# Tung-I/Dual-awareness-Attention-for-Few-shot-Object-Detection

Measured on AMD Instinct MI355X. Metric: query-images/sec (res50, way=2, shot=3, bs=4 per GPU, train-mode forward), higher is better.
Workload: dtype f32 (operands, accumulation, results; multiplies as an exact bf16x3 split, six bf16 MFMA products each)

## Files before the change

dual-awareness-attention-for-few-shot-object-detection_amd/csrc/igemm.hip:

```cpp
#include "common.h"
#include "../../include/dana_hip_debug.h"
#include <stdlib.h>
#include <atomic>

namespace {

typedef float f32x16 __attribute__((ext_vector_type(16)));
typedef unsigned int u32x4 __attribute__((ext_vector_type(4)));

struct IgemmParams {
  const float* A;
  const float* Bw;
  float* C;
  const float* scale;
  const float* shift;
  const float* residual;
  const float* mask;
  long ldm;
  int M, N, K;
  int IH, IW, OH, OW, Cin, KH, KW, stride, pad;
  int M0, IH1, IW1, OH1, OW1, pix1;
  float* C1;
  const float* residual1;
  long ldc1, ldr1;
  int lda, ldb;
  long ldc, ldr;
  long batch_a, batch_b, batch_c;
  unsigned a_bytes, b_bytes;
  float alpha;
  int relu;
  int vec_io;
  int vec_ss;
  int tiles_m, tiles_n;
  const float* A2;
  int lda2, IH2, IW2, stride2, K1;
  int IH21, IW21, pix21;
  int bpre;
  const void* Bw2;
  const float* scale2;
  const float* shift2;
  int N2, relu2;
  unsigned a2_bytes;
  int apre, a_rows;
  int res_sample, res_h, res_w, res_oh, res_ow;
  unsigned res_bytes;
  unsigned long long* trace;
};

constexpr int BK = 32;
constexpr int LDS_LD = 36;
constexpr unsigned OOB = 0x80000000u;

__device__ __forceinline__ int xcd_remap(int bid, int nwg) {
  const int q = nwg / 8, r = nwg % 8;
  const int xcd = bid % 8, local = bid / 8;
  return (xcd < r ? xcd * (q + 1) : r * (q + 1) + (xcd - r) * q) + local;
}

__device__ __forceinline__ float4 ldg_b128(__amdgpu_buffer_rsrc_t r, unsigned off) {
  u32x4 v = __builtin_amdgcn_raw_buffer_load_b128(r, (int)off, 0, 0);
  return *(float4*)&v;
}

template <int BM, int BN, int STEM>
__global__ void __launch_bounds__(256, 2) igemm_f32_kernel(IgemmParams p) {
  constexpr int TM = BM / 64, TN = BN / 64;
  constexpr int RA = BM / 32, RB = BN / 32;
  constexpr int CLD = BN + 4;
  extern __shared__ __attribute__((aligned(16))) float smem[];
  float* As = smem;
  float* Bs = smem + 2 * BM * LDS_LD;

  const int tid = threadIdx.x;
  const int lane = tid & 63, wave = tid >> 6;
  const int wm = wave >> 1, wn = wave & 1;
  const int li = lane & 31, lh = lane >> 5;

  const int vid = xcd_remap((int)(blockIdx.z * gridDim.x + blockIdx.x), (int)(gridDim.x * gridDim.z));
  const int zb = vid / (int)gridDim.x;
  const int tile = vid - zb * (int)gridDim.x;
  const int tm_idx = tile / p.tiles_n, tn_idx = tile % p.tiles_n;
  const int m0 = tm_idx * BM, n0 = tn_idx * BN;
  const float* Ab = p.A + (long)zb * p.batch_a;
  const float* Bb = p.Bw + (long)zb * p.batch_b;
  float* Cb = p.C + (long)zb * p.batch_c;
  const __amdgpu_buffer_rsrc_t ra_src = __builtin_amdgcn_make_buffer_rsrc((void*)Ab, 0, (int)p.a_bytes, 0x00020000);
  const __amdgpu_buffer_rsrc_t rb_src = __builtin_amdgcn_make_buffer_rsrc((void*)Bb, 0, (int)p.b_bytes, 0x00020000);

  const int c4 = tid & 7;
  const int r0 = tid >> 3;
  unsigned a_off[RA];
  unsigned long long a_mask[RA];
  bool a_seg1[RA];
#pragma unroll
  for (int j = 0; j < RA; ++j) {
    const int m = m0 + r0 + 32 * j;
    const bool ok = m < p.M;
    const bool s1 = ok && m >= p.M0;
    a_seg1[j] = s1;
    const int mm = ok ? (s1 ? m - p.M0 : m) : 0;
    const int IH = s1 ? p.IH1 : p.IH, IW = s1 ? p.IW1 : p.IW, OW = s1 ? p.OW1 : p.OW;
    const int ohw = (s1 ? p.OH1 : p.OH) * OW;
    const int img = mm / ohw, rem = mm - img * ohw;
    const int oh = rem / OW, ow = rem - oh * OW;
    const int ih0 = oh * p.stride - p.pad, iw0 = ow * p.stride - p.pad;
    const int pix = (s1 ? p.pix1 : 0) + (img * IH + ih0) * IW;
    unsigned long long mask = 0;
    if (STEM) {
      const int iw = iw0 + c4;
      if (ok && c4 < 7 && iw >= 0 && iw < IW)
        for (int kh = 0; kh < 7; ++kh)
          if (ih0 + kh >= 0 && ih0 + kh < IH) mask |= 1ull << kh;
      a_off[j] = (unsigned)((pix + iw) * 16);
    } else {
      if (ok)
        for (int kh = 0; kh < p.KH; ++kh)
          for (int kw = 0; kw < p.KW; ++kw)
            if (ih0 + kh >= 0 && ih0 + kh < IH && iw0 + kw >= 0 && iw0 + kw < IW)
              mask |= 1ull << (kh * p.KW + kw);
      a_off[j] = (unsigned)(((pix + iw0) * p.lda + c4 * 4) * 4);
    }
    a_mask[j] = mask;
  }
  unsigned b_off[RB];
#pragma unroll
  for (int j = 0; j < RB; ++j) {
    const int n = n0 + r0 + 32 * j;
    b_off[j] = n < p.N ? (unsigned)((n * p.ldb + c4 * 4) * 4) : OOB;
  }

  float4 ra0[RA], rb0[RB], ra1[RA], rb1[RB];
  auto load_tile = [&](int kt, float4(&ra)[RA], float4(&rb)[RB]) {
    const int k0 = kt * BK;
    const bool kok = (k0 + c4 * 4) < p.K;
    int tap;
    unsigned delta, delta1;
    if (STEM) {
      tap = kt;
      delta = (unsigned)(kt * p.IW * 16);
      delta1 = (unsigned)(kt * p.IW1 * 16);
    } else {
      tap = k0 / p.Cin;
      const int cin0 = k0 - tap * p.Cin;
      const int kh = tap / p.KW, kw = tap - kh * p.KW;
      delta = (unsigned)(((kh * p.IW + kw) * p.lda + cin0) * 4);
      delta1 = (unsigned)(((kh * p.IW1 + kw) * p.lda + cin0) * 4);
    }
#pragma unroll
    for (int j = 0; j < RA; ++j) {
      const bool ok = kok && ((a_mask[j] >> tap) & 1ull);
      ra[j] = ldg_b128(ra_src, ok ? a_off[j] + (a_seg1[j] ? delta1 : delta) : OOB);
    }
#pragma unroll
    for (int j = 0; j < RB; ++j) rb[j] = ldg_b128(rb_src, (kok && b_off[j] != OOB) ? b_off[j] + k0 * 4 : OOB);
  };
  auto store_tile = [&](int buf, const float4(&ra)[RA], const float4(&rb)[RB]) {
    float* as = As + buf * BM * LDS_LD;
    float* bs = Bs + buf * BN * LDS_LD;
#pragma unroll
    for (int j = 0; j < RA; ++j) *(float4*)(as + (r0 + 32 * j) * LDS_LD + c4 * 4) = ra[j];
#pragma unroll
    for (int j = 0; j < RB; ++j) *(float4*)(bs + (r0 + 32 * j) * LDS_LD + c4 * 4) = rb[j];
  };

  f32x16 acc[TM][TN];
#pragma unroll
  for (int i = 0; i < TM; ++i)
#pragma unroll
// ... 215 lines not shown
             : __builtin_amdgcn_make_buffer_rsrc((void*)(p.residual ? (seg1 ? p.residual1 : p.residual) + mrel * ld_r : p.A), 0,
                                                 p.residual ? rows_valid * ldr4 : 0, 0x00020000);
    const __amdgpu_buffer_rsrc_t rc_msk = __builtin_amdgcn_make_buffer_rsrc(
        (void*)(p.mask ? p.mask + (long)m0 * p.ldm : p.A), 0, p.mask ? rows_valid * ldm4 : 0, 0x00020000);
    const int lrow = wm * (BM / 2) + 4 * lh;
    unsigned vo_c[TN], vo_r[TN], vo_m[TN];
#pragma unroll
    for (int j = 0; j < TN; ++j) {
      const bool nok = ncol[j] < p.N;
      vo_c[j] = nok ? (unsigned)(lrow * ldc4 + ncol[j] * 4) : OOB;
      vo_r[j] = nok ? (unsigned)((RSMP ? 0 : lrow * ldr4) + ncol[j] * 4) : OOB;
      vo_m[j] = nok ? (unsigned)(lrow * ldm4 + ncol[j] * 4) : OOB;
    }
    auto run = [&](auto res_c, auto relu_c, auto mask_c) {
      constexpr bool RES = decltype(res_c)::value != 0, RELU = decltype(relu_c)::value != 0, MASK = decltype(mask_c)::value != 0;
      constexpr int HI = (MASK || HALVES) ? 1 : TM;
#pragma unroll
      for (int i0 = 0; i0 < TM; i0 += HI) {
        float res[RES ? HI : 1][TN][16], msk[MASK ? HI : 1][TN][16];
#pragma unroll
        for (int ii = 0; ii < HI; ++ii)
#pragma unroll
          for (int j = 0; j < TN; ++j)
#pragma unroll
            for (int r = 0; r < 16; ++r) {
              const int rt = (i0 + ii) * 32 + (r & 3) + 8 * (r >> 2);
              if constexpr (RES && RSMP)
                res[ii][j][r] = __builtin_bit_cast(float, __builtin_amdgcn_raw_buffer_load_b32(rc_res, (int)(vo_r[j] + rtab[lrow + rt]), 0, 0));
              else if constexpr (RES)
                res[ii][j][r] = __builtin_bit_cast(float, __builtin_amdgcn_raw_buffer_load_b32(rc_res, (int)(vo_r[j] + (unsigned)(rt * ldr4)), 0, 0));
              if constexpr (MASK)
                msk[ii][j][r] = __builtin_bit_cast(float, __builtin_amdgcn_raw_buffer_load_b32(rc_msk, (int)(vo_m[j] + (unsigned)(rt * ldm4)), 0, 0));
            }
#pragma unroll
        for (int ii = 0; ii < HI; ++ii)
#pragma unroll
          for (int j = 0; j < TN; ++j)
#pragma unroll
            for (int r = 0; r < 16; ++r) {
              const int rt = (i0 + ii) * 32 + (r & 3) + 8 * (r >> 2);
              float v = acc[i0 + ii][j][r] * scv[j] + shv[j];
              if constexpr (RES) v += res[ii][j][r];
              if constexpr (RELU) v = fmaxf(v, 0.f);
              if constexpr (MASK) v = msk[ii][j][r] > 0.f ? v : 0.f;
              __builtin_amdgcn_raw_buffer_store_b32(__builtin_bit_cast(unsigned, v), rc_dst, (int)(vo_c[j] + (unsigned)(rt * ldc4)), 0, 0);
            }
      }
    };
    if (WITH_MASK && p.mask) {
      if (p.residual) {
        if (p.relu) run(IC<1>{}, IC<1>{}, IC<1>{});
        else run(IC<1>{}, IC<0>{}, IC<1>{});
      } else {
        if (p.relu) run(IC<0>{}, IC<1>{}, IC<1>{});
        else run(IC<0>{}, IC<0>{}, IC<1>{});
      }
    } else if (p.residual) {
      if (p.relu) run(IC<1>{}, IC<1>{}, IC<0>{});
      else run(IC<1>{}, IC<0>{}, IC<0>{});
    } else {
      if (p.relu) run(IC<0>{}, IC<1>{}, IC<0>{});
      else run(IC<0>{}, IC<0>{}, IC<0>{});
    }
  } else {
#pragma unroll
    for (int i = 0; i < TM; ++i)
#pragma unroll
      for (int j = 0; j < TN; ++j)
#pragma unroll
        for (int r = 0; r < 16; ++r) {
          const int m = m0 + wm * (BM / 2) + i * 32 + (r & 3) + 8 * (r >> 2) + 4 * lh;
          if (m < p.M && ncol[j] < p.N) {
            const bool s1 = m >= p.M0;
            float v = acc[i][j][r] * scv[j] + shv[j];
            if (p.residual) v += s1 ? p.residual1[(long)(m - p.M0) * p.ldr1 + ncol[j]] : p.residual[(long)m * p.ldr + ncol[j]];
            if (p.relu) v = fmaxf(v, 0.f);
            if (p.mask && !(p.mask[(long)m * p.ldm + ncol[j]] > 0.f)) v = 0.f;
            (s1 ? p.C1 + (long)(m - p.M0) * p.ldc1 : Cb + (long)m * p.ldc)[ncol[j]] = v;
          }
        }
  }
}

template <int BM, int BN, int STEM, int BPRE = 0, int FUSE = 0, int ELDS = 0, int RSMP = 0>
__device__ __forceinline__ void igemm_split_body(const IgemmParams& p) {
  static_assert(!RSMP || (!STEM && !FUSE && !ELDS), "sampled residual: register epilogue of the plain conv / GEMM forms");
  constexpr int TM = BM / 64, TN = BN / 64;
  constexpr int RA = BM / 64;
  constexpr int RB = BPRE ? (3 * BN * 2 + 255) / 256 : BN / 64;
  constexpr int CLD = BN + 4;
  extern __shared__ __attribute__((aligned(16))) float smem[];
  unsigned* As = (unsigned*)smem;
  unsigned* Bs = As + 2 * 3 * BM * SLD;

  const int tid = threadIdx.x;
  const int lane = tid & 63, wave = tid >> 6;
  const int wm = wave >> 1, wn = wave & 1;
  const int li = lane & 31, lh = lane >> 5;

  const unsigned long long t_start = p.trace ? __builtin_readcyclecounter() : 0ull;
  const unsigned long long w_start = p.trace ? wall_clock64() : 0ull;
  const int vid = xcd_remap((int)(blockIdx.z * gridDim.x + blockIdx.x), (int)(gridDim.x * gridDim.z));
  const int zb = vid / (int)gridDim.x;
  const int tile = vid - zb * (int)gridDim.x;
  const int tm_idx = tile / p.tiles_n, tn_idx = tile % p.tiles_n;
  const int m0 = tm_idx * BM, n0 = tn_idx * BN;
  const float* Ab = p.A + (long)zb * p.batch_a;
  const float* Bb = p.Bw + (long)zb * p.batch_b;
  float* Cb = p.C + (long)zb * p.batch_c;
  __amdgpu_buffer_rsrc_t ra_src = __builtin_amdgcn_make_buffer_rsrc((void*)Ab, 0, (int)p.a_bytes, 0x00020000);
  const __amdgpu_buffer_rsrc_t rb_src = __builtin_amdgcn_make_buffer_rsrc((void*)Bb, 0, (int)p.b_bytes, 0x00020000);

  int cin_t = STEM ? SBK : p.Cin;
  const int kw_t = STEM ? 2 : p.KW;
  const int kh_t = STEM ? 7 : p.KH;
  const int lda4 = (STEM ? 4 : p.lda) * 4;
  const int kwstep = STEM ? 4 * lda4 : lda4;
  const int c4 = tid & 3;
  const int r0 = tid >> 2;
  const int wcol = ((c4 >> 1) ^ swz(r0)) * 4 + (c4 & 1) * 2;
  const int rcol = (lh ^ swz(li)) * 4;
  const int klim = p.K - c4 * 4;
  constexpr int DEAD = (int)0x80000000;
  unsigned a_off[RA];
  unsigned a_mask[RA];
  int a_dseg[RA];
  unsigned a_off2[RA];
  const bool lin = !STEM && p.KH * p.KW == 1 && p.stride == 1 && p.pad == 0;
#pragma unroll
  for (int j = 0; j < RA; ++j) {
    const int m = m0 + r0 + 64 * j;
    const bool ok = m < p.M;
    const bool s1 = ok && m >= p.M0;
    const int mm = ok ? (s1 ? m - p.M0 : m) : 0;
    if (lin && !p.A2) {
      a_off[j] = (unsigned)(((s1 ? p.pix1 : 0) + mm) * lda4 + c4 * 16);
      a_mask[j] = ok ? 1u : 0u;
      a_dseg[j] = 0;
      a_off2[j] = OOB;
      continue;
    }
    const int IH = s1 ? p.IH1 : p.IH, IW = s1 ? p.IW1 : p.IW, OW = s1 ? p.OW1 : p.OW;
    const int ohw = (s1 ? p.OH1 : p.OH) * OW;
    const int img = mm / ohw, rem = mm - img * ohw;
    const int oh = rem / OW, ow = rem - oh * OW;
    const int ih0 = oh * p.stride - p.pad, iw0 = ow * p.stride - p.pad;
    const int pix = (s1 ? p.pix1 : 0) + (img * IH + ih0) * IW;
    unsigned mask = 0;
    if (STEM) {
      const int lo = ih0 < 0 ? -ih0 : 0, hi = IH - ih0 < 7 ? IH - ih0 : 7;
      const int iwa = iw0 + c4, iwb = iw0 + 4 + c4;
      const unsigned cv = ((iwa >= 0 && iwa < IW) ? 0x1555u : 0u) | ((iwb >= 0 && iwb < IW && c4 < 3) ? 0x2aaau : 0u);
      if (ok && hi > lo) mask = ((1u << (2 * hi)) - (1u << (2 * lo))) & cv;
    } else if (ok) {
      unsigned colbits = 0;
      for (int kw = 0; kw < kw_t; ++kw)
        if (iw0 + kw >= 0 && iw0 + kw < IW) colbits |= 1u << kw;
      for (int kh = 0; kh < kh_t; ++kh)
        if (ih0 + kh >= 0 && ih0 + kh < IH) mask |= colbits << (kh * kw_t);
    }
    a_off[j] = STEM ? (unsigned)((pix + iw0 + c4) * lda4) : (unsigned)((pix + iw0) * lda4 + c4 * 16);
    a_mask[j] = mask;
    a_dseg[j] = s1 ? (p.IW1 - p.IW) * lda4 : 0;
    a_off2[j] = (!STEM && p.A2 && ok)
                    ? (unsigned)(((s1 ? p.pix21 : 0) + ((long)img * (s1 ? p.IH21 : p.IH2) + oh * p.stride2) * (s1 ? p.IW21 : p.IW2) +
                                  ow * p.stride2) * p.lda2 * 4 + c4 * 16)
                    : OOB;
  }
  unsigned b_cur[RB];
  int b_lim[RB];
  int b_lds[RB];
#pragma unroll
  for (int j = 0; j < RB; ++j) {
    if constexpr (BPRE) {
      const int q = (tid + 256 * j < 6 * BN) ? tid + 256 * j : tid;
      const int pl = q / (2 * BN), rem = q - pl * (2 * BN);
      const int row = rem >> 1, half = rem & 1;
      const int n = n0 + row;
      b_cur[j] = (unsigned)((((long)pl * p.N + n) * SBK + half * 8) * 2);
      b_lim[j] = n < p.N ? (p.K + SBK - 1) / SBK * SBK : DEAD;
      b_lds[j] = (pl * BN + row) * SLD + (half ^ swz(row)) * 4;
    } else {
      const int n = n0 + r0 + 64 * j;
      b_cur[j] = (unsigned)((n * p.ldb + c4 * 4) * 4);
      b_lim[j] = n < p.N ? klim : DEAD;
      b_lds[j] = 0;
    }
  }
  const unsigned B_STEP = BPRE ? (unsigned)p.N * 3u * SBK * 2u : SBK * 4;

  float4 ra0[RA], rb0[RB], ra1[RA], rb1[RB];
  int lt_k0 = 0, lt_cin = 0, lt_kh = 0, lt_kw = 0;
// ... 481 lines not shown
          *(float4*)(c_base + (long)(qq * RPP) * ld_c) = make_float4(v[0], v[1], v[2], v[3]);
        }
      }
    };
    if (p.mask) {
      if (p.residual) {
        if (p.relu) emit(IC<1>{}, IC<1>{}, IC<1>{});
        else emit(IC<1>{}, IC<0>{}, IC<1>{});
      } else {
        if (p.relu) emit(IC<0>{}, IC<1>{}, IC<1>{});
        else emit(IC<0>{}, IC<0>{}, IC<1>{});
      }
    } else if (p.residual) {
      if (p.relu) emit(IC<1>{}, IC<1>{}, IC<0>{});
      else emit(IC<1>{}, IC<0>{}, IC<0>{});
    } else {
      if (p.relu) emit(IC<0>{}, IC<1>{}, IC<0>{});
      else emit(IC<0>{}, IC<0>{}, IC<0>{});
    }
  } else if (full4) {
#pragma unroll
    for (int q = 0; q < NP; ++q) {
      const int rr = er + q * RPP;
      const int m = m0 + rr;
      if (m < p.M) {
        const float4 a4 = *(const float4*)(Cs + rr * CLD + ec);
        float v[4] = {a4.x * sc[0] + sh[0], a4.y * sc[1] + sh[1], a4.z * sc[2] + sh[2], a4.w * sc[3] + sh[3]};
        float* cp = c_base + (long)(q * RPP) * ld_c;
        if (!one_seg) {
          const bool s1 = m >= p.M0;
          cp = s1 ? p.C1 + (long)(m - p.M0) * p.ldc1 + n : Cb + (long)m * p.ldc + n;
        }
        if (p.residual) {
          v[0] += rres[q].x;
          v[1] += rres[q].y;
          v[2] += rres[q].z;
          v[3] += rres[q].w;
        }
        if (p.relu) {
#pragma unroll
          for (int t = 0; t < 4; ++t) v[t] = fmaxf(v[t], 0.f);
        }
        if (p.mask) {
          const float4 k4 = *(const float4*)(p.mask + (long)m * p.ldm + n);
          v[0] = k4.x > 0.f ? v[0] : 0.f;
          v[1] = k4.y > 0.f ? v[1] : 0.f;
          v[2] = k4.z > 0.f ? v[2] : 0.f;
          v[3] = k4.w > 0.f ? v[3] : 0.f;
        }
        *(float4*)cp = make_float4(v[0], v[1], v[2], v[3]);
      }
    }
  } else {
    for (int q = 0; q < NP; ++q) {
      const int rr = er + q * RPP;
      const int m = m0 + rr;
      if (m >= p.M) break;
      const bool s1 = m >= p.M0;
      float* cp = s1 ? p.C1 + (long)(m - p.M0) * p.ldc1 + n : Cb + (long)m * p.ldc + n;
      const float* rp = s1 ? p.residual1 + (long)(m - p.M0) * p.ldr1 + n : p.residual + (long)m * p.ldr + n;
      for (int t = 0; t < 4; ++t)
        if ((n + t) < p.N) {
          float x = Cs[rr * CLD + ec + t] * sc[t] + sh[t];
          if (p.residual) x += rp[t];
          if (p.relu) x = fmaxf(x, 0.f);
          if (p.mask && !(p.mask[(long)m * p.ldm + n + t] > 0.f)) x = 0.f;
          cp[t] = x;
        }
    }
  }
  if (p.trace && tid == 0) {
    unsigned long long* tr = p.trace + ((long)blockIdx.z * gridDim.x + blockIdx.x) * 8;
    tr[0] = t_start;
    tr[1] = t_loop;
    tr[2] = t_loop_end;
    tr[3] = __builtin_readcyclecounter();
    tr[4] = (unsigned long long)__builtin_amdgcn_s_getreg((31 << 11) | 4) | ((unsigned long long)__builtin_amdgcn_s_getreg((31 << 11) | 20) << 32);
    tr[5] = wall_clock64();
    tr[6] = w_start;
    tr[7] = 0;
  }
}

template <int BM, int BN, int STEM, int BPRE = 0, int FUSE = 0, int ELDS = 0, int RSMP = 0>
__global__ void __launch_bounds__(256, 2) igemm_split_kernel(IgemmParams p) {
  igemm_split_body<BM, BN, STEM, BPRE, FUSE, ELDS, RSMP>(p);
}
template <int STEM, int BPRE, int ELDS, int RSMP = 0>
__global__ void __launch_bounds__(256, 1) __attribute__((amdgpu_num_vgpr(192))) igemm_split_kernel_128(IgemmParams p) {
  igemm_split_body<128, 128, STEM, BPRE, 0, ELDS, RSMP>(p);
}

template <int BN, int NST, int APRE, int DF = 0>
__global__ void __launch_bounds__(256, NST == 2 ? 3 : (NST == 3 ? 2 : 1)) igemm_dma_kernel(IgemmParams p) {
  static_assert(APRE || NST == 2, "fp32 activation rows: two stages");
  static_assert(!DF || (APRE && NST >= 3), "two fragment sets: planes x planes, three or more stages");
  constexpr int BM = 128, TM = 2, TN = BN / 64;
  constexpr int STAGE_B = 3 * (BM + BN) * 32;
  constexpr int NPB = 3 * BN / 32, PB = (NPB + 3) / 4;
  constexpr int NDMA = (APRE ? 3 : 0) + PB;
  constexpr int AHEAD = NST == 2 ? 2 : NST - 1;
  constexpr int RA = BM / 64;
  extern __shared__ __attribute__((aligned(16))) float smem[];
  const int tid = threadIdx.x;
  const int lane = tid & 63, wave = __builtin_amdgcn_readfirstlane(tid >> 6);
  const int wm = wave >> 1, wn = wave & 1;
  const int li = lane & 31, lh = lane >> 5;
  const unsigned long long t_start = p.trace ? __builtin_readcyclecounter() : 0ull;
  const unsigned long long w_start = p.trace ? wall_clock64() : 0ull;
  const int vid = xcd_remap((int)(blockIdx.z * gridDim.x + blockIdx.x), (int)(gridDim.x * gridDim.z));
  const int zb = vid / (int)gridDim.x;
  const int tile = vid - zb * (int)gridDim.x;
  const int tm_idx = tile / p.tiles_n, tn_idx = tile % p.tiles_n;
  const int m0 = tm_idx * BM, n0 = tn_idx * BN;
  float* Cb = p.C + (long)zb * p.batch_c;
  __amdgpu_buffer_rsrc_t ra_src =
      __builtin_amdgcn_make_buffer_rsrc((void*)(p.A + (long)zb * p.batch_a), 0, (int)p.a_bytes, 0x00020000);
  const __amdgpu_buffer_rsrc_t rb_src =
      __builtin_amdgcn_make_buffer_rsrc((void*)(p.Bw + (long)zb * p.batch_b), 0, (int)p.b_bytes, 0x00020000);
  const int nk = (p.K + SBK - 1) / SBK;

  const int prow = lane >> 1, phalf = (lane & 1) ^ ((lane >> 4) & 1);
  const int arow = m0 + 32 * wave + prow;
  const unsigned a_vo = arow < p.M ? (unsigned)(arow * 32 + phalf * 16) : OOB;
  const unsigned a_pstride = (unsigned)p.a_rows * 32u, b_pstride = (unsigned)p.N * 32u;
  unsigned b_vo[PB];
  int b_pl[PB], b_lds[PB];
#pragma unroll
  for (int j = 0; j < PB; ++j) {
    int q = wave + 4 * j;
    if (q >= NPB) q -= 4;
    const int pl = q / (BN / 32), rg = q % (BN / 32);
    const int n = n0 + 32 * rg + prow;
    b_vo[j] = n < p.N ? (unsigned)(n * 32 + phalf * 16) : OOB;
    b_pl[j] = pl;
    b_lds[j] = 3 * BM * 32 + (pl * BN + 32 * rg) * 32;
  }
  typedef __attribute__((address_space(3))) void lds_void;
  typedef __attribute__((address_space(3))) char lds_char;
  lds_char* const lds0 = (lds_char*)(lds_void*)smem;
  auto issue = [&](int t, int stage) {
    const bool live = t < nk;
    lds_char* base = lds0 + stage * STAGE_B;
    if constexpr (APRE) {
      const unsigned av = live ? a_vo : OOB;
      const unsigned sa = (unsigned)t * 3u * a_pstride;
#pragma unroll
      for (int pl = 0; pl < 3; ++pl)
        __builtin_amdgcn_raw_ptr_buffer_load_lds(ra_src, (lds_void*)(base + (pl * BM + 32 * wave) * 32), 16, (int)av,
                                                 (int)(sa + pl * a_pstride), 0, 0);
    }
    const unsigned sb = (unsigned)t * 3u * b_pstride;
#pragma unroll
    for (int j = 0; j < PB; ++j)
      __builtin_amdgcn_raw_ptr_buffer_load_lds(rb_src, (lds_void*)(base + b_lds[j]), 16, (int)(live ? b_vo[j] : OOB),
                                               (int)(sb + b_pl[j] * b_pstride), 0, 0);
  };

  int cin_t = p.Cin;
  const int kw_t = p.KW, kh_t = p.KH;
  const int lda4 = p.lda * 4;
  const int c4 = tid & 3, r0 = tid >> 2;
  const int wcol = ((c4 >> 1) ^ swz(r0)) * 4 + (c4 & 1) * 2;
  const int klim = p.K - c4 * 4;
  constexpr int DEAD = (int)0x80000000;
  unsigned a_off[RA], a_mask[RA], a_off2[RA];
  int a_dseg[RA];
  int lt_k0 = 0, lt_cin = 0, lt_kh = 0, lt_kw = 0;
  unsigned lt_bit = 1u;
  unsigned a_cur[RA];
  int a_lim[RA];
  if constexpr (!APRE) {
    const bool lin = p.KH * p.KW == 1 && p.stride == 1 && p.pad == 0;
#pragma unroll
    for (int j = 0; j < RA; ++j) {
      const int m = m0 + r0 + 64 * j;
      const bool ok = m < p.M;
      const bool s1 = ok && m >= p.M0;
      const int mm = ok ? (s1 ? m - p.M0 : m) : 0;
      if (lin && !p.A2) {
        a_off[j] = (unsigned)(((s1 ? p.pix1 : 0) + mm) * lda4 + c4 * 16);
        a_mask[j] = ok ? 1u : 0u;
        a_dseg[j] = 0;
        a_off2[j] = OOB;
      } else {
        const int IH = s1 ? p.IH1 : p.IH, IW = s1 ? p.IW1 : p.IW, OW = s1 ? p.OW1 : p.OW;
        const int ohw = (s1 ? p.OH1 : p.OH) * OW;
        const int img = mm / ohw, rem = mm - img * ohw;
        const int oh = rem / OW, ow = rem - oh * OW;
        const int ih0 = oh * p.stride - p.pad, iw0 = ow * p.stride - p.pad;
        const int pix = (s1 ? p.pix1 : 0) + (img * IH + ih0) * IW;
        unsigned mask = 0;
        if (ok) {
          unsigned colbits = 0;
          for (int kw = 0; kw < kw_t; ++kw)
            if (iw0 + kw >= 0 && iw0 + kw < IW) colbits |= 1u << kw;
          for (int kh = 0; kh < kh_t; ++kh)
            if (ih0 + kh >= 0 && ih0 + kh < IH) mask |= colbits << (kh * kw_t);
        }
        a_off[j] = (unsigned)((pix + iw0) * lda4 + c4 * 16);
        a_mask[j] = mask;
        a_dseg[j] = s1 ? (p.IW1 - p.IW) * lda4 : 0;
// ... 180 lines not shown
  const unsigned long long t_loop_end = p.trace ? __builtin_readcyclecounter() : 0ull;
  epilogue_regs<BM, BN, (NST == 2 && BN == 128) ? 1 : 0, 0>(p, acc, m0, n0, Cb, wm, wn, li, lh);
  if (p.trace && tid == 0) {
    unsigned long long* tr = p.trace + ((long)blockIdx.z * gridDim.x + blockIdx.x) * 8;
    tr[0] = t_start;
    tr[1] = t_loop;
    tr[2] = t_loop_end;
    tr[3] = __builtin_readcyclecounter();
    tr[4] = (unsigned long long)__builtin_amdgcn_s_getreg((31 << 11) | 4) | ((unsigned long long)__builtin_amdgcn_s_getreg((31 << 11) | 20) << 32);
    tr[5] = wall_clock64();
    tr[6] = w_start;
    tr[7] = 0;
  }
}

template <int NMAX>
__global__ void __launch_bounds__(256)
gemm_skinny_kernel(const float* __restrict__ a, const float* __restrict__ b, float* __restrict__ c,
                   const float* __restrict__ scale, const float* __restrict__ shift, int M, int N, int K, long lda,
                   long ldb, long ldc, float alpha, int relu) {
  const int lane = threadIdx.x & 63;
  const long m = (long)blockIdx.x * 4 + (threadIdx.x >> 6);
  if (m >= M) return;
  float acc[NMAX];
#pragma unroll
  for (int n = 0; n < NMAX; ++n) acc[n] = 0.f;
  const float4* ar = (const float4*)(a + m * lda);
  for (int k4 = lane; k4 < K / 4; k4 += 64) {
    const float4 x = ar[k4];
#pragma unroll
    for (int n = 0; n < NMAX; ++n)
      if (n < N) {
        const float4 w = ((const float4*)(b + n * ldb))[k4];
        acc[n] += x.x * w.x + x.y * w.y + x.z * w.z + x.w * w.w;
      }
  }
#pragma unroll
  for (int n = 0; n < NMAX; ++n) {
#pragma unroll
    for (int o = 32; o > 0; o >>= 1) acc[n] += __shfl_xor(acc[n], o);
  }
  if (lane == 0)
    for (int n = 0; n < N; ++n) {
      float v = acc[n] * alpha * (scale ? scale[n] : 1.f) + (shift ? shift[n] : 0.f);
      if (relu) v = fmaxf(v, 0.f);
      c[m * ldc + n] = v;
    }
}

__global__ void __launch_bounds__(256)
split_weight_kernel(const float* __restrict__ w, long ldw, long batch_w, int n, int k, int kp,
                    unsigned short* __restrict__ out) {
  const int kq = kp / 4;
  const long idx = (long)blockIdx.x * blockDim.x + threadIdx.x;
  if (idx >= (long)n * kq) return;
  const int row = (int)(idx / kq), k4 = (int)(idx - (long)row * kq) * 4;
  const float* src = w + blockIdx.y * batch_w + (long)row * ldw + k4;
  float4 v = make_float4(0.f, 0.f, 0.f, 0.f);
  if (k4 + 3 < k) v = *(const float4*)src;
  else {
    if (k4 < k) v.x = src[0];
    if (k4 + 1 < k) v.y = src[1];
    if (k4 + 2 < k) v.z = src[2];
  }
  uint2 h, m, l;
  split3(v, h, m, l);
  const int ks = k4 / SBK, kk = k4 - ks * SBK;
  unsigned short* o = out + blockIdx.y * 3 * (long)n * kp + (((long)ks * 3) * n + row) * SBK + kk;
  *(uint2*)o = h;
  *(uint2*)(o + (long)n * SBK) = m;
  *(uint2*)(o + 2 * (long)n * SBK) = l;
}

std::atomic<int>& epilogue_mode_cell() {
  static std::atomic<int> cell(0);
  return cell;
}

std::atomic<int> g_last_form(0);
constexpr int form_code(int family, int bm, int bn, int stem, int bpre, int fuse, int elds, int nst, int apre, int df) {
  return family | (bm / 64) << 4 | (bn / 64) << 6 | stem << 8 | bpre << 9 | fuse << 10 | elds << 11 | nst << 12 | apre << 16 | df << 17;
}

template <int BM, int BN, int STEM>
int launch(const IgemmParams& p0, int batch, hipStream_t s) {
  g_last_form.store(form_code(DANA_IGEMM_FAMILY_F32, BM, BN, STEM, 0, 0, 0, 0, 0, 0), std::memory_order_relaxed);
  IgemmParams p = p0;
  p.tiles_m = (p.M + BM - 1) / BM;
  p.tiles_n = (p.N + BN - 1) / BN;
  size_t lds = (size_t)2 * (BM + BN) * LDS_LD * sizeof(float);
  const size_t lds_c = (size_t)BM * (BN + 4) * sizeof(float);
  if (lds_c > lds) lds = lds_c;
  static DeviceOnce attr;
  attr.once([&] { return hipFuncSetAttribute((const void*)igemm_f32_kernel<BM, BN, STEM>, hipFuncAttributeMaxDynamicSharedMemorySize, (int)lds); });
  dim3 grid(p.tiles_m * p.tiles_n, 1, batch);
  igemm_f32_kernel<BM, BN, STEM><<<grid, 256, lds, s>>>(p);
  return 0;
}

template <int BM, int BN, int STEM = 0, int BPRE = 0, int FUSE = 0, int ELDS = 0, int RSMP = 0>
int launch_split(const IgemmParams& p0, int batch, hipStream_t s) {
  if constexpr (BPRE == 0 && FUSE == 0) {
    if (p0.bpre) return launch_split<BM, BN, STEM, 1, 0, ELDS, RSMP>(p0, batch, s);
  }
  if constexpr (ELDS == 0 && FUSE == 0 && RSMP == 0) {
    if (epilogue_mode_cell().load(std::memory_order_relaxed)) return launch_split<BM, BN, STEM, BPRE, 0, 1>(p0, batch, s);
  }
  g_last_form.store(form_code(BM * BN >= 128 * 128 ? DANA_IGEMM_FAMILY_SPLIT_128 : DANA_IGEMM_FAMILY_SPLIT, BM, BN, STEM, BPRE, FUSE ? 1 : 0,
                              ELDS, 0, 0, 0), std::memory_order_relaxed);
  IgemmParams p = p0;
  p.tiles_m = (p.M + BM - 1) / BM;
  p.tiles_n = (p.N + BN - 1) / BN;
  size_t lds = (size_t)2 * 3 * (BM + BN) * SLD * sizeof(unsigned);
  const size_t lds_c = (size_t)BM * (BN + 4) * sizeof(float);
  if (lds_c > lds && ELDS) lds = lds_c;
  if (FUSE && lds < (size_t)4 * 3 * BM * 16 * 2) lds = (size_t)4 * 3 * BM * 16 * 2;
  if (FUSE == 2 || RSMP) lds += (size_t)BM * 4;
  dim3 grid(p.tiles_m * p.tiles_n, 1, batch);
  static DeviceOnce attr;
  if constexpr (BM * BN >= 128 * 128) {
    attr.once([&] { return hipFuncSetAttribute((const void*)igemm_split_kernel_128<STEM, BPRE, ELDS, RSMP>, hipFuncAttributeMaxDynamicSharedMemorySize,
                                (int)lds); });
    igemm_split_kernel_128<STEM, BPRE, ELDS, RSMP><<<grid, 256, lds, s>>>(p);
  } else {
    attr.once([&] { return hipFuncSetAttribute((const void*)igemm_split_kernel<BM, BN, STEM, BPRE, FUSE, ELDS, RSMP>,
                                hipFuncAttributeMaxDynamicSharedMemorySize, (int)lds); });
    igemm_split_kernel<BM, BN, STEM, BPRE, FUSE, ELDS, RSMP><<<grid, 256, lds, s>>>(p);
  }
  return 0;
}

template <int BN, int NST, int APRE, int DF = 0>
int launch_dma(const IgemmParams& p0, int batch, hipStream_t s) {
  g_last_form.store(form_code(DANA_IGEMM_FAMILY_DMA, 128, BN, 0, 1, 0, 0, NST, APRE, DF), std::memory_order_relaxed);
  IgemmParams p = p0;
  p.tiles_m = (p.M + 127) / 128;
  p.tiles_n = (p.N + BN - 1) / BN;
  const size_t lds = (size_t)NST * 3 * (128 + BN) * 32;
  static DeviceOnce attr;
  attr.once([&] { return hipFuncSetAttribute((const void*)igemm_dma_kernel<BN, NST, APRE, DF>, hipFuncAttributeMaxDynamicSharedMemorySize, (int)lds); });
  dim3 grid(p.tiles_m * p.tiles_n, 1, batch);
  igemm_dma_kernel<BN, NST, APRE, DF><<<grid, 256, lds, s>>>(p);
  return 0;
}

std::atomic<int>& mfma_mode_cell() {
  static std::atomic<int> cell(getenv("DANA_MFMA_SPLIT") ? atoi(getenv("DANA_MFMA_SPLIT")) : 1);
  return cell;
}
int env_choice(const char* name, std::initializer_list<int> allowed) {
  const char* e = getenv(name);
  if (!e || !*e) return -1;
  const int v = atoi(e);
  for (int a : allowed)
    if (a == v) return v;
  fprintf(stderr, "libdana_hip: %s=%s is not one of the accepted values; ignored\n", name, e);
  return -1;
}
int dma_kernel_env() {
  static const int v = env_choice("DANA_DMA_KERNEL", {0, 1, 2});
  return v;
}
std::atomic<int>& dma_kernel_cell() {
  static std::atomic<int> cell(dma_kernel_env());
  return cell;
}
int pp_stages_env() {
  static const int v = env_choice("DANA_PP_STAGES", {2, 3, 4, 6, 13, 14});
  return v;
}
std::atomic<int>& pp_stages_cell() {
  static std::atomic<int> cell(pp_stages_env());
  return cell;
}
unsigned long long* g_trace = nullptr;

int dispatch_sampled(const IgemmParams& p, int batch, hipStream_t s) {
  const int mode = mfma_mode_cell().load(std::memory_order_relaxed);
  if (!mode || p.apre || p.mask || p.KH * p.KW > 32 || p.M0 != p.M || epilogue_mode_cell().load(std::memory_order_relaxed)) return -1;
  if (p.N <= 64) return -1;
  if (mode == 3) return launch_split<64, 64, 0, 0, 0, 0, 1>(p, batch, s);
  if (mode == 4) return launch_split<128, 128, 0, 0, 0, 0, 1>(p, batch, s);
  if (p.N <= 256 && p.N % 128 != 0 && p.N % 128 <= 32) return launch_split<64, 64, 0, 0, 0, 0, 1>(p, batch, s);
  const long t128 = (long)((p.M + 127) / 128) * ((p.N + 127) / 128) * batch;
  if (t128 < 100) return launch_split<64, 64, 0, 0, 0, 0, 1>(p, batch, s);
  return launch_split<128, 128, 0, 0, 0, 0, 1>(p, batch, s);
}

int dispatch(const IgemmParams& p, int batch, int stem, hipStream_t s) {
  if (p.res_sample) return stem ? -1 : dispatch_sampled(p, batch, s);
  if (stem) {
    const int smode = mfma_mode_cell().load(std::memory_order_relaxed);
    return smode ? launch_split<128, 64, 1>(p, batch, s) : launch<128, 64, 1>(p, batch, s);
  }
  const int mode = mfma_mode_cell().load(std::memory_order_relaxed);
  if (p.apre) {
    const int pp_env = pp_stages_cell().load(std::memory_order_relaxed);
    const long t128 = (long)((p.M + 127) / 128) * ((p.N + 127) / 128) * batch;
    const int stages = pp_env >= 0 ? pp_env : ((t128 < 400 || p.K >= 1024) ? 13 : 2);
    if (p.N <= 64) return stages == 2 ? launch_dma<64, 2, 1>(p, batch, s) : launch_dma<64, 3, 1>(p, batch, s);
    if (stages == 2) return launch_dma<128, 2, 1>(p, batch, s);
    if (stages == 4) return launch_dma<128, 4, 1>(p, batch, s);
    if (stages == 6) return launch_dma<128, 6, 1>(p, batch, s);
    if (stages == 13) return launch_dma<128, 3, 1, 1>(p, batch, s);
    if (stages == 14) return launch_dma<128, 4, 1, 1>(p, batch, s);
    return launch_dma<128, 3, 1>(p, batch, s);
  }
  if (mode == 1 && p.bpre && !p.mask && p.KH * p.KW <= 32) {
    const int dm_env = dma_kernel_cell().load(std::memory_order_relaxed);
    const int dm = dm_env >= 0 ? dm_env : 1;
    if (dm == 2) return p.N <= 64 ? launch_dma<64, 2, 0>(p, batch, s) : launch_dma<128, 2, 0>(p, batch, s);
    if (dm == 1 && p.N > 64) {
      const long t128 = (long)((p.M + 127) / 128) * ((p.N + 127) / 128) * batch;
      if (t128 >= 600 && p.K <= 192) return launch_dma<128, 2, 0>(p, batch, s);
    }
  }
  if (mode && p.KH * p.KW <= 32) {
    if (mode == 2) return launch_split<128, 64>(p, batch, s);
    if (mode == 3) return launch_split<64, 64>(p, batch, s);
    if (mode == 4) return launch_split<128, 128>(p, batch, s);
    if (mode == 5) return launch_split<64, 128>(p, batch, s);
    if (p.N <= 64) return launch_split<128, 64>(p, batch, s);
    if (mode == 1 && p.N <= 256 && p.N % 128 != 0 && p.N % 128 <= 32) return launch_split<64, 64>(p, batch, s);
    const long t128 = (long)((p.M + 127) / 128) * ((p.N + 127) / 128) * batch;
    if (mode == 1 && t128 < 100) return launch_split<64, 64>(p, batch, s);
    return launch_split<128, 128>(p, batch, s);
  }
  return launch<64, 64, 0>(p, batch, s);
}

int run(IgemmParams& p, int batch, int stem, hipStream_t s) {
  if (p.M0 <= 0 || p.M0 > p.M) p.M0 = p.M;
  if (p.M0 == p.M) {
    p.IH1 = p.IH; p.IW1 = p.IW; p.OH1 = p.OH; p.OW1 = p.OW; p.pix1 = 0;
    p.C1 = p.C; p.ldc1 = p.ldc; p.residual1 = p.residual; p.ldr1 = p.ldr;
  }
  p.trace = g_trace;
  p.vec_io = (p.ldc % 4 == 0) && (((uintptr_t)p.C & 15) == 0) && (p.batch_c % 4 == 0) &&
             (!p.residual || ((p.ldr % 4 == 0) && (((uintptr_t)p.residual & 15) == 0))) &&
             (p.ldc1 % 4 == 0) && (((uintptr_t)p.C1 & 15) == 0) &&
             (!p.residual1 || ((p.ldr1 % 4 == 0) && (((uintptr_t)p.residual1 & 15) == 0)));
  p.vec_ss = (((uintptr_t)p.scale | (uintptr_t)p.shift) & 15) == 0;
  return dispatch(p, batch, stem, s);
}

}

extern "C" {

int dana_set_epilogue_mode(int mode) {
  DANA_CHECK_ARG(mode == 0 || mode == 1, "dana_set_epilogue_mode: 0 (accumulator registers) or 1 (LDS C tile)");
  epilogue_mode_cell().store(mode, std::memory_order_relaxed);
  return DANA_OK;
}
int dana_get_epilogue_mode(void) { return epilogue_mode_cell().load(std::memory_order_relaxed); }

int dana_set_mfma_mode(int mode) {
  DANA_CHECK_ARG(mode == 0 || mode == 1, "dana_set_mfma_mode: mode must be 0 (f32 MFMA) or 1 (bf16x6 split)");
  mfma_mode_cell().store(mode, std::memory_order_relaxed);
  return DANA_OK;
}

int dana_debug_force_tile(int tile) {
  DANA_CHECK_ARG(tile == 0 || (tile >= 2 && tile <= 5), "dana_debug_force_tile: 0 (dispatcher), 2 = 128x64, 3 = 64x64, 4 = 128x128, 5 = 64x128");
  DANA_CHECK_ARG(mfma_mode_cell().load(std::memory_order_relaxed) != 0, "dana_debug_force_tile: split kernel only");
  mfma_mode_cell().store(tile ? tile : 1, std::memory_order_relaxed);
  return DANA_OK;
}

int dana_debug_set_dma_kernel(int v) {
  DANA_CHECK_ARG(v >= -1 && v <= 2, "dana_debug_set_dma_kernel: -1 (environment / default), 0 (split kernel), 1 (measured rule) or 2 (wherever it runs)");
  dma_kernel_cell().store(v < 0 ? dma_kernel_env() : v, std::memory_order_relaxed);
// ... 277 lines not shown
  IgemmParams p;
  memset(&p, 0, sizeof(p));
  p.A = a0;
  p.Bw = weight;
  p.C = out0;
  p.scale = scale;
  p.shift = shift;
  p.residual = residual;
  p.IH = p.OH = oh0;
  p.IW = p.OW = ow0;
  p.M0 = (int)m0;
  p.M = (int)(m0 + m1);
  if (n1) {
    p.IH1 = p.OH1 = oh1;
    p.IW1 = p.OW1 = ow1;
    p.pix1 = (int)m0;
    p.C1 = out1;
    p.IH21 = h1;
    p.IW21 = w1;
    p.pix21 = n0 * h0 * w0;
  }
  p.N = cout;
  p.KH = p.KW = 1;
  p.stride = 1;
  p.pad = 0;
  p.Cin = k0;
  p.K = k0 + k1;
  p.lda = (int)lda0;
  p.ldb = p.K;
  p.a_bytes = (unsigned)a0_bytes;
  p.b_bytes = (unsigned)b_bytes;
  p.bpre = bpre;
  p.A2 = a1;
  p.lda2 = (int)lda1;
  p.IH2 = h0;
  p.IW2 = w0;
  p.stride2 = stride1;
  p.K1 = k1;
  p.a2_bytes = (unsigned)a1_bytes;
  p.ldc = out0_pix_stride > 0 ? out0_pix_stride : cout;
  p.ldr = res_pix_stride > 0 ? res_pix_stride : cout;
  p.ldc1 = n1 ? (out1_pix_stride > 0 ? out1_pix_stride : cout) : p.ldc;
  p.ldr1 = p.ldr;
  p.alpha = 1.f;
  p.relu = (flags & DANA_EPI_RELU) ? 1 : 0;
  p.ldm = cout;
  run(p, 1, 0, (hipStream_t)stream);
  DANA_CHECK_LAUNCH(who);
  return DANA_OK;
}

int dana_conv1x1_cat2_nhwc(const float* a0, long a0_pix_stride, int k0, const float* a1, long a1_pix_stride, int k1,
                           int batch, int h1, int w1, int stride1, const float* weight, float* output,
                           const float* scale, const float* shift, const float* residual, long out_pix_stride,
                           long res_pix_stride, int cout, int flags, dana_stream_t stream) {
  return cat2_impl("dana_conv1x1_cat2_nhwc", a0, a0_pix_stride, k0, a1, a1_pix_stride, k1, batch, h1, w1, 0, 0, 0, stride1,
                   weight, output, nullptr, scale, shift, residual, out_pix_stride, 0, res_pix_stride, cout, flags, stream);
}

int dana_conv1x1_cat2_nhwc_dual(const float* a0, long a0_pix_stride, int k0, const float* a1, long a1_pix_stride, int k1,
                                int n0, int h0, int w0, int n1, int h1, int w1, int stride1, const float* weight,
                                float* out0, float* out1, const float* scale, const float* shift, long out0_pix_stride,
                                long out1_pix_stride, int cout, int flags, dana_stream_t stream) {
  return cat2_impl("dana_conv1x1_cat2_nhwc_dual", a0, a0_pix_stride, k0, a1, a1_pix_stride, k1, n0, h0, w0, n1, h1, w1,
                   stride1, weight, out0, out1, scale, shift, nullptr, out0_pix_stride, out1_pix_stride, 0, cout, flags, stream);
}

size_t dana_split_weight_bytes(int n, int k, int batch) {
  if (n <= 0 || k <= 0 || batch <= 0) return 0;
  return (size_t)batch * 3 * n * ((k + SBK - 1) / SBK * SBK) * 2;
}

int dana_split_weight(const float* w, long ldw, int n, int k, int batch, long batch_w, void* out, dana_stream_t stream) {
  DANA_CHECK_ARG(n > 0 && k > 0 && batch > 0 && ldw >= k, "dana_split_weight: bad shape");
  DANA_CHECK_ARG(w && out && ((uintptr_t)w & 15) == 0 && ((uintptr_t)out & 15) == 0 && ldw % 4 == 0 && batch_w % 4 == 0,
                 "dana_split_weight: pointers / strides must be 16-byte aligned");
  const int kp = (k + SBK - 1) / SBK * SBK;
  dim3 grid((unsigned)dana_ceil_div((long)n * (kp / 4), 256), batch);
  split_weight_kernel<<<grid, 256, 0, (hipStream_t)stream>>>(w, ldw, batch_w, n, k, kp, (unsigned short*)out);
  DANA_CHECK_LAUNCH("dana_split_weight");
  return DANA_OK;
}

int dana_gemm_nt(const float* a, const float* b, float* c, const float* scale, const float* shift,
                 const float* residual, int m, int n, int k, long lda, long ldb, long ldc, long ldr, int batch,
                 long batch_a, long batch_b, long batch_c, float alpha, int flags, dana_stream_t stream) {
  DANA_CHECK_ARG(m >= 0 && n >= 0 && k > 0 && batch >= 0, "dana_gemm_nt: bad shape m=%d n=%d k=%d", m, n, k);
  if (m == 0 || n == 0 || batch == 0) return DANA_OK;
  DANA_CHECK_ARG(a && b && c, "dana_gemm_nt: null pointer");
  DANA_CHECK_ARG(k % 4 == 0 && lda % 4 == 0 && ldb % 4 == 0 && batch_a % 4 == 0 && batch_b % 4 == 0,
                 "dana_gemm_nt: k, lda, ldb and batch strides must be multiples of 4 (16-byte rows)");
  const int bpre = (flags & DANA_W_SPLIT3) ? 1 : 0;
  DANA_CHECK_ARG(!bpre || (dana_get_mfma_mode() != 0 && ldb % SBK == 0 && ldb >= k && batch_b % 8 == 0 && n > 8),
                 "dana_gemm_nt: DANA_W_SPLIT3 needs the split kernel, ldb = k rounded up to 16, n > 8");
  const int apre = (flags & DANA_A_SPLIT3) ? 1 : 0;
  DANA_CHECK_ARG(!apre || (bpre && lda % SBK == 0 && lda >= k && batch_a % 8 == 0),
                 "dana_gemm_nt: DANA_A_SPLIT3 needs DANA_W_SPLIT3 too, lda = k rounded up to 16");
  DANA_CHECK_ARG(lda >= k && ldb >= k && ldc >= n, "dana_gemm_nt: leading dimension smaller than the row");
  DANA_CHECK_ARG(((uintptr_t)a & 15) == 0 && ((uintptr_t)b & 15) == 0, "dana_gemm_nt: a/b must be 16-byte aligned");
  DANA_CHECK_ARG(!residual || batch == 1, "dana_gemm_nt: residual only with batch == 1");
  hipStream_t s = (hipStream_t)stream;
  if (n <= 8 && batch == 1 && !residual) {
    gemm_skinny_kernel<8><<<dana_ceil_div(m, 4), 256, 0, s>>>(a, b, c, scale, shift, m, n, k, lda, ldb, ldc, alpha,
                                                              (flags & DANA_EPI_RELU) ? 1 : 0);
    DANA_CHECK_LAUNCH("dana_gemm_nt(skinny)");
    return DANA_OK;
  }
  const long a_bytes = apre ? (long)3 * m * lda * 2 : ((long)(m - 1) * lda + k) * 4;
  const long b_bytes = bpre ? (long)3 * n * ldb * 2 : ((long)(n - 1) * ldb + k) * 4;
  DANA_CHECK_ARG(a_bytes < (long)OOB && b_bytes < (long)OOB, "dana_gemm_nt: operand slice >= 2 GiB; split it");
  IgemmParams p;
  memset(&p, 0, sizeof(p));
  p.A = a;
  p.Bw = b;
  p.C = c;
  p.scale = scale;
  p.shift = shift;
  p.residual = residual;
  p.M = m;
  p.N = n;
  p.K = k;
  p.IH = m;
  p.IW = 1;
  p.OH = m;
  p.OW = 1;
  p.Cin = (k + BK - 1) / BK * BK;
  p.KH = p.KW = 1;
  p.stride = 1;
  p.pad = 0;
  p.lda = (int)lda;
  p.ldb = (int)ldb;
  p.a_bytes = (unsigned)a_bytes;
  p.b_bytes = (unsigned)b_bytes;
  p.ldc = ldc;
  p.ldr = ldr > 0 ? ldr : ldc;
  p.batch_a = apre ? batch_a / 2 : batch_a;
  p.batch_b = bpre ? batch_b / 2 : batch_b;
  p.apre = apre;
  p.a_rows = m;
  p.batch_c = batch_c;
  p.bpre = bpre;
  p.alpha = alpha;
  p.relu = (flags & DANA_EPI_RELU) ? 1 : 0;
  run(p, batch, 0, s);
  DANA_CHECK_LAUNCH("dana_gemm_nt");
  return DANA_OK;
}

}
```

dual-awareness-attention-for-few-shot-object-detection_amd/csrc/winograd.hip:

```cpp
#include "common.h"
#include "../../include/dana_hip.h"

namespace {

typedef unsigned int u32x4 __attribute__((ext_vector_type(4)));
constexpr unsigned OOB = 0x80000000u;

__device__ __forceinline__ float4 f4add(float4 a, float4 b) { return make_float4(a.x + b.x, a.y + b.y, a.z + b.z, a.w + b.w); }
__device__ __forceinline__ float4 f4sub(float4 a, float4 b) { return make_float4(a.x - b.x, a.y - b.y, a.z - b.z, a.w - b.w); }

__global__ void __launch_bounds__(256)
wino_filter_kernel(const float* __restrict__ w, float* __restrict__ U, int cout, int cin) {
  const long i = (long)blockIdx.x * blockDim.x + threadIdx.x;
  if (i >= (long)cout * cin) return;
  const int ci = (int)(i % cin);
  const long co = i / cin;
  float g[3][3];
#pragma unroll
  for (int r = 0; r < 3; ++r)
#pragma unroll
    for (int c = 0; c < 3; ++c) g[r][c] = w[((co * 3 + r) * 3 + c) * cin + ci];
  float t[4][3];
#pragma unroll
  for (int c = 0; c < 3; ++c) {
    t[0][c] = g[0][c];
    t[1][c] = 0.5f * (g[0][c] + g[1][c] + g[2][c]);
    t[2][c] = 0.5f * (g[0][c] - g[1][c] + g[2][c]);
    t[3][c] = g[2][c];
  }
#pragma unroll
  for (int r = 0; r < 4; ++r) {
    const float u0 = t[r][0], u1 = 0.5f * (t[r][0] + t[r][1] + t[r][2]), u2 = 0.5f * (t[r][0] - t[r][1] + t[r][2]),
                u3 = t[r][2];
    const long plane = (long)cout * cin;
    U[(r * 4 + 0) * plane + i] = u0;
    U[(r * 4 + 1) * plane + i] = u1;
    U[(r * 4 + 2) * plane + i] = u2;
    U[(r * 4 + 3) * plane + i] = u3;
  }
}

__global__ void __launch_bounds__(256)
wino_input_kernel(const float* __restrict__ in, float* __restrict__ V, int H, int W, int C4, int th, int tw,
                  long tiles, int lda, unsigned in_bytes) {
  const long idx = (long)blockIdx.x * blockDim.x + threadIdx.x;
  if (idx >= tiles * C4) return;
  const int c4 = (int)(idx % C4);
  const long t = idx / C4;
  const int j = (int)(t % tw);
  const int i = (int)((t / tw) % th);
  const int img = (int)(t / ((long)tw * th));
  const __amdgpu_buffer_rsrc_t src = __builtin_amdgcn_make_buffer_rsrc((void*)in, 0, (int)in_bytes, 0x00020000);
  float4 d[4][4];
#pragma unroll
  for (int r = 0; r < 4; ++r) {
    const int y = 2 * i - 1 + r;
#pragma unroll
    for (int c = 0; c < 4; ++c) {
      const int x = 2 * j - 1 + c;
      const bool ok = y >= 0 && y < H && x >= 0 && x < W;
      const unsigned off = ok ? (unsigned)((((img * H + y) * W + x) * lda + c4 * 4) * 4) : OOB;
      u32x4 v = __builtin_amdgcn_raw_buffer_load_b128(src, (int)off, 0, 0);
      d[r][c] = *(float4*)&v;
    }
  }
  float4 tm[4][4];
#pragma unroll
  for (int c = 0; c < 4; ++c) {
    tm[0][c] = f4sub(d[0][c], d[2][c]);
    tm[1][c] = f4add(d[1][c], d[2][c]);
    tm[2][c] = f4sub(d[2][c], d[1][c]);
    tm[3][c] = f4sub(d[1][c], d[3][c]);
  }
  const long plane = tiles * (long)C4;
  float4* out = (float4*)V + t * C4 + c4;
#pragma unroll
  for (int r = 0; r < 4; ++r) {
    out[(r * 4 + 0) * plane] = f4sub(tm[r][0], tm[r][2]);
    out[(r * 4 + 1) * plane] = f4add(tm[r][1], tm[r][2]);
    out[(r * 4 + 2) * plane] = f4sub(tm[r][2], tm[r][1]);
    out[(r * 4 + 3) * plane] = f4sub(tm[r][1], tm[r][3]);
  }
}

__global__ void __launch_bounds__(256)
wino_output_kernel(const float* __restrict__ M, float* __restrict__ out, const float* __restrict__ scale,
                   const float* __restrict__ shift, const float* __restrict__ mask, long ldm, int H, int W, int N4,
                   int th, int tw, long tiles, long ldc, int relu, const float* __restrict__ res = nullptr, long ldr = 0,
// ... 15 lines not shown
  float4 s[2][4];
#pragma unroll
  for (int c = 0; c < 4; ++c) {
    s[0][c] = f4add(f4add(m[0][c], m[1][c]), m[2][c]);
    s[1][c] = f4sub(f4sub(m[1][c], m[2][c]), m[3][c]);
  }
  const float4 sc = scale ? ((const float4*)scale)[n4] : make_float4(1, 1, 1, 1);
  const float4 sh = shift ? ((const float4*)shift)[n4] : make_float4(0, 0, 0, 0);
#pragma unroll
  for (int r = 0; r < 2; ++r) {
    const int y = 2 * i + r;
    if (y >= H) break;
    float4 y0 = f4add(f4add(s[r][0], s[r][1]), s[r][2]);
    float4 y1 = f4sub(f4sub(s[r][1], s[r][2]), s[r][3]);
    float4 o[2] = {y0, y1};
#pragma unroll
    for (int c = 0; c < 2; ++c) {
      const int x = 2 * j + c;
      if (x >= W) break;
      float4 v = make_float4(o[c].x * sc.x + sh.x, o[c].y * sc.y + sh.y, o[c].z * sc.z + sh.z, o[c].w * sc.w + sh.w);
      if (res) {
        const float4 q = *(const float4*)(res + (((img / rgroup) * H + y) * W + x) * ldr + n4 * 4);
        v = f4add(v, q);
      }
      if (relu) v = make_float4(fmaxf(v.x, 0.f), fmaxf(v.y, 0.f), fmaxf(v.z, 0.f), fmaxf(v.w, 0.f));
      if (mask) {
        const float4 k = *(const float4*)(mask + ((img * H + y) * W + x) * ldm + n4 * 4);
        v = make_float4(k.x > 0.f ? v.x : 0.f, k.y > 0.f ? v.y : 0.f, k.z > 0.f ? v.z : 0.f, k.w > 0.f ? v.w : 0.f);
      }
      *(float4*)(out + ((img * H + y) * W + x) * ldc + n4 * 4) = v;
    }
  }
}

__device__ __forceinline__ float4 f4s(float4 a, float s) { return make_float4(a.x * s, a.y * s, a.z * s, a.w * s); }
__device__ __forceinline__ float4 f4ma(float4 a, float s, float4 b) {
  return make_float4(a.x * s + b.x, a.y * s + b.y, a.z * s + b.z, a.w * s + b.w);
}

__device__ __forceinline__ void bt6(const float4 (&d)[6], float4 (&o)[6]) {
  o[0] = f4add(f4ma(d[2], -5.f, f4s(d[0], 4.f)), d[4]);
  o[1] = f4add(f4ma(f4add(d[1], d[2]), -4.f, d[3]), d[4]);
  o[2] = f4add(f4ma(f4sub(d[1], d[2]), 4.f, f4sub(d[4], d[3])), make_float4(0.f, 0.f, 0.f, 0.f));
  o[3] = f4add(f4ma(f4sub(d[3], d[1]), 2.f, f4sub(d[4], d[2])), make_float4(0.f, 0.f, 0.f, 0.f));
  o[4] = f4add(f4ma(f4sub(d[1], d[3]), 2.f, f4sub(d[4], d[2])), make_float4(0.f, 0.f, 0.f, 0.f));
  o[5] = f4add(f4ma(d[3], -5.f, f4s(d[1], 4.f)), d[5]);
}

__global__ void __launch_bounds__(256)
wino4_filter_kernel(const float* __restrict__ w, float* __restrict__ U, int cout, int cin) {
  const long i = (long)blockIdx.x * blockDim.x + threadIdx.x;
  if (i >= (long)cout * cin) return;
  const int ci = (int)(i % cin);
  const long co = i / cin;
  float g[3][3];
#pragma unroll
  for (int r = 0; r < 3; ++r)
#pragma unroll
    for (int c = 0; c < 3; ++c) g[r][c] = w[((co * 3 + r) * 3 + c) * cin + ci];
  float t[6][3];
#pragma unroll
  for (int c = 0; c < 3; ++c) {
    const float a = g[0][c], b = g[1][c], d = g[2][c];
    t[0][c] = 0.25f * a;
    t[1][c] = -(a + b + d) * (1.f / 6.f);
    t[2][c] = (-a + b - d) * (1.f / 6.f);
    t[3][c] = a * (1.f / 24.f) + b * (1.f / 12.f) + d * (1.f / 6.f);
    t[4][c] = a * (1.f / 24.f) - b * (1.f / 12.f) + d * (1.f / 6.f);
    t[5][c] = d;
  }
  const long plane = (long)cout * cin;
#pragma unroll
  for (int r = 0; r < 6; ++r) {
    const float a = t[r][0], b = t[r][1], d = t[r][2];
    U[(r * 6 + 0) * plane + i] = 0.25f * a;
    U[(r * 6 + 1) * plane + i] = -(a + b + d) * (1.f / 6.f);
    U[(r * 6 + 2) * plane + i] = (-a + b - d) * (1.f / 6.f);
    U[(r * 6 + 3) * plane + i] = a * (1.f / 24.f) + b * (1.f / 12.f) + d * (1.f / 6.f);
    U[(r * 6 + 4) * plane + i] = a * (1.f / 24.f) - b * (1.f / 12.f) + d * (1.f / 6.f);
    U[(r * 6 + 5) * plane + i] = d;
  }
}

__global__ void __launch_bounds__(256)
wino4_input_kernel(const float* __restrict__ in, float* __restrict__ V, int H, int W, int C4, int th, int tw,
                   long tiles, int lda, unsigned in_bytes, long plane_tiles = 0, long tile_off = 0) {
  if (plane_tiles == 0) plane_tiles = tiles;
  const unsigned idx = blockIdx.x * blockDim.x + threadIdx.x;
  if (idx >= (unsigned)(tiles * C4)) return;
  const unsigned t = idx / (unsigned)C4;
  const int c4 = (int)(idx - t * (unsigned)C4);
  const unsigned tr = t / (unsigned)tw;
  const int j = (int)(t - tr * (unsigned)tw);
  const int img = (int)(tr / (unsigned)th);
  const int i = (int)(tr - (unsigned)img * (unsigned)th);
  const __amdgpu_buffer_rsrc_t src = __builtin_amdgcn_make_buffer_rsrc((void*)in, 0, (int)in_bytes, 0x00020000);
  float4 tm[6][6];
#pragma unroll
  for (int c = 0; c < 6; ++c) {
    const int x = 4 * j - 1 + c;
    float4 col[6], o[6];
#pragma unroll
    for (int r = 0; r < 6; ++r) {
      const int y = 4 * i - 1 + r;
      const bool ok = y >= 0 && y < H && x >= 0 && x < W;
      const unsigned off = ok ? (unsigned)((((img * H + y) * W + x) * lda + c4 * 4) * 4) : OOB;
      u32x4 v = __builtin_amdgcn_raw_buffer_load_b128(src, (int)off, 0, 0);
      col[r] = *(float4*)&v;
    }
    bt6(col, o);
#pragma unroll
    for (int r = 0; r < 6; ++r) tm[r][c] = o[r];
  }
  const long plane = plane_tiles * (long)C4;
  float4* out = (float4*)V + (tile_off + t) * C4 + c4;
#pragma unroll
  for (int r = 0; r < 6; ++r) {
    float4 o[6];
    bt6(tm[r], o);
#pragma unroll
    for (int c = 0; c < 6; ++c) out[(r * 6 + c) * plane] = o[c];
  }
}

__device__ __forceinline__ void at6(const float4 (&m)[6], float4 (&o)[4]) {
  const float4 p = f4add(m[1], m[2]), q = f4sub(m[1], m[2]), r = f4add(m[3], m[4]), s = f4sub(m[3], m[4]);
  o[0] = f4add(f4add(m[0], p), r);
  o[1] = f4ma(s, 2.f, q);
  o[2] = f4ma(r, 4.f, p);
  o[3] = f4add(f4ma(s, 8.f, q), m[5]);
}

template <int SUB = 1>
__global__ void __launch_bounds__(256)
wino4_output_kernel(const float* __restrict__ M, float* __restrict__ out, const float* __restrict__ scale,
                    const float* __restrict__ shift, const float* __restrict__ mask, long ldm, int H, int W, int N4,
                    int th, int tw, long tiles, long ldc, int relu, long plane_tiles = 0, long tile_off = 0,
                    const float* __restrict__ res = nullptr, long ldr = 0, int rgroup = 1) {
  const unsigned idx = blockIdx.x * blockDim.x + threadIdx.x;
  if (idx >= (unsigned)(tiles * N4)) return;
  if (plane_tiles == 0) plane_tiles = tiles;
  const unsigned t = idx / (unsigned)N4;
  const int n4 = (int)(idx - t * (unsigned)N4);
  const unsigned tr = t / (unsigned)tw;
  const int j = (int)(t - tr * (unsigned)tw);
  const long img = (long)(tr / (unsigned)th);
  const int i = (int)(tr - (unsigned)img * (unsigned)th);
  const long plane = plane_tiles * (long)N4;
  const float4* mp = (const float4*)M + tile_off * N4 + (long)idx;
  float4 s[4][6];
#pragma unroll
  for (int c = 0; c < 6; ++c) {
    float4 col[6], o[4];
#pragma unroll
    for (int r = 0; r < 6; ++r) col[r] = mp[(r * 6 + c) * plane];
    at6(col, o);
#pragma unroll
    for (int r = 0; r < 4; ++r) s[r][c] = o[r];
  }
  const float4 sc = scale ? ((const float4*)scale)[n4] : make_float4(1, 1, 1, 1);
  const float4 sh = shift ? ((const float4*)shift)[n4] : make_float4(0, 0, 0, 0);
#pragma unroll
  for (int r = 0; r < 4; r += SUB) {
    const int y = 4 * i + r;
    if (y >= H) break;
    float4 o[4];
    at6(s[r], o);
#pragma unroll
    for (int c = 0; c < 4; c += SUB) {
      const int x = 4 * j + c;
      if (x >= W) break;
      float4 v = make_float4(o[c].x * sc.x + sh.x, o[c].y * sc.y + sh.y, o[c].z * sc.z + sh.z, o[c].w * sc.w + sh.w);
      if constexpr (SUB == 2) {
        if (relu) v = make_float4(fmaxf(v.x, 0.f), fmaxf(v.y, 0.f), fmaxf(v.z, 0.f), fmaxf(v.w, 0.f));
        *(float4*)(out + ((img * ((H + 1) / 2) + y / 2) * ((W + 1) / 2) + x / 2) * ldc + n4 * 4) = v;
        continue;
      }
      if (res) {
        const float4 q = *(const float4*)(res + (((img / rgroup) * H + y) * W + x) * ldr + n4 * 4);
        v = f4add(v, q);
      }
      if (relu) v = make_float4(fmaxf(v.x, 0.f), fmaxf(v.y, 0.f), fmaxf(v.z, 0.f), fmaxf(v.w, 0.f));
      if (mask) {
        const float4 k = *(const float4*)(mask + ((img * H + y) * W + x) * ldm + n4 * 4);
        v = make_float4(k.x > 0.f ? v.x : 0.f, k.y > 0.f ? v.y : 0.f, k.z > 0.f ? v.z : 0.f, k.w > 0.f ? v.w : 0.f);
      }
      *(float4*)(out + ((img * H + y) * W + x) * ldc + n4 * 4) = v;
    }
  }
}

__device__ __forceinline__ void a4to6(const float4 (&y)[4], float4 (&o)[6]) {
  const float4 p = f4add(y[0], y[2]), q = f4add(y[1], y[3]);
  const float4 r = f4ma(y[2], 4.f, y[0]), t = f4ma(y[3], 8.f, f4s(y[1], 2.f));
  o[0] = y[0];
  o[1] = f4add(p, q);
  o[2] = f4sub(p, q);
  o[3] = f4add(r, t);
  o[4] = f4sub(r, t);
  o[5] = y[3];
}

__global__ void __launch_bounds__(256)
wino4_outgrad_kernel(const float* __restrict__ dy, float* __restrict__ dM, int H, int W, int N4, int th, int tw,
// ... 164 lines not shown

static int wgrad_winograd4_impl(const float* grad_out, const float* input, const float* v_saved, float* grad_weight,
                                int batch, int h, int w, int cin, int cout, long in_pix_stride, long grad_pix_stride,
                                const float* row_scale, int accumulate, void* workspace, size_t workspace_bytes,
                                dana_stream_t stream);

int dana_conv3x3_wgrad_winograd4(const float* grad_out, const float* input, float* grad_weight, int batch, int h, int w,
                                 int cin, int cout, long in_pix_stride, long grad_pix_stride, const float* row_scale,
                                 int accumulate, void* workspace, size_t workspace_bytes, dana_stream_t stream) {
  DANA_CHECK_ARG(input || batch == 0, "dana_conv3x3_wgrad_winograd4: null pointer");
  return wgrad_winograd4_impl(grad_out, input, nullptr, grad_weight, batch, h, w, cin, cout, in_pix_stride, grad_pix_stride,
                              row_scale, accumulate, workspace, workspace_bytes, stream);
}

int dana_conv3x3_wgrad_winograd4_v(const float* grad_out, const float* v, float* grad_weight, int batch, int h, int w,
                                   int cin, int cout, long grad_pix_stride, const float* row_scale, int accumulate,
                                   void* workspace, size_t workspace_bytes, dana_stream_t stream) {
  DANA_CHECK_ARG(v || batch == 0, "dana_conv3x3_wgrad_winograd4_v: null pointer");
  DANA_CHECK_ARG(((uintptr_t)v & 15) == 0, "dana_conv3x3_wgrad_winograd4_v: v must be 16-byte aligned");
  return wgrad_winograd4_impl(grad_out, nullptr, v, grad_weight, batch, h, w, cin, cout, 0, grad_pix_stride, row_scale,
                              accumulate, workspace, workspace_bytes, stream);
}

static int wgrad_winograd4_impl(const float* grad_out, const float* input, const float* v_saved, float* grad_weight,
                                int batch, int h, int w, int cin, int cout, long in_pix_stride, long grad_pix_stride,
                                const float* row_scale, int accumulate, void* workspace, size_t workspace_bytes,
                                dana_stream_t stream) {
  DANA_CHECK_ARG(batch >= 0 && h > 0 && w > 0 && cin > 0 && cout > 0 && cin % 64 == 0 && cout % 4 == 0,
                 "dana_conv3x3_wgrad_winograd4: bad shape (cin %% 64, cout %% 4)");
  if (batch == 0) return DANA_OK;
  DANA_CHECK_ARG(grad_out && (input || v_saved) && grad_weight, "dana_conv3x3_wgrad_winograd4: null pointer");
  const long lda = in_pix_stride > 0 ? in_pix_stride : cin;
  const long ldy = grad_pix_stride > 0 ? grad_pix_stride : cout;
  DANA_CHECK_ARG(lda % 4 == 0 && ldy % 4 == 0 && ((uintptr_t)input & 15) == 0 && ((uintptr_t)grad_out & 15) == 0,
                 "dana_conv3x3_wgrad_winograd4: strides / pointers must be 16-byte aligned");
  const long in_bytes = (long)batch * h * w * lda * 4;
  DANA_CHECK_ARG(in_bytes < (long)OOB, "dana_conv3x3_wgrad_winograd4: input span >= 2 GiB; split the batch");
  const size_t need = dana_conv3x3_wgrad_winograd4_workspace_bytes(batch, h, w, cin, cout);
  if (!workspace || workspace_bytes < need) {
    dana_set_error("dana_conv3x3_wgrad_winograd4: workspace %zu < %zu", workspace_bytes, need);
    return DANA_ERR_WORKSPACE;
  }
  const WinoPlan p = wino_plan(batch, h, w, cin, cout, 4);
  hipStream_t s = (hipStream_t)stream;
  const float* V = v_saved ? v_saved : (const float*)workspace;
  float* dM = (float*)((char*)workspace + p.v_bytes);
  float* dU = (float*)((char*)workspace + p.total);
  const size_t du = dana_align_up((size_t)36 * cout * cin * 4, 256);
  void* gws = (char*)workspace + p.total + du;
  const int C4 = cin / 4, N4 = cout / 4;
  DANA_CHECK_ARG(p.tiles * (long)(C4 > N4 ? C4 : N4) < (1L << 31), "dana_conv3x3_wgrad_winograd4: too many tiles x channels");
  if (!v_saved) {
    wino4_input_kernel<<<dana_ceil_div(p.tiles * C4, 256), 256, 0, s>>>(input, (float*)workspace, h, w, C4, p.th, p.tw, p.tiles,
                                                                       (int)lda, (unsigned)in_bytes);
    DANA_CHECK_LAUNCH("dana_conv3x3_wgrad_winograd4(input transform)");
  }
  wino4_outgrad_kernel<<<dana_ceil_div(p.tiles * N4, 256), 256, 0, s>>>(grad_out, dM, h, w, N4, p.th, p.tw, p.tiles, ldy);
  DANA_CHECK_LAUNCH("dana_conv3x3_wgrad_winograd4(output-gradient transform)");
  int rc = dana_wgrad_tn_batched(dM, V, dU, 36, (int)p.tiles, cout, cin, p.tiles * cout, p.tiles * cin, gws,
                                 workspace_bytes - (p.total + du), (void*)s);
  if (rc) return rc;
  const long total = (long)cout * cin;
  wino4_filtergrad_kernel<<<dana_ceil_div(total, 256), 256, 0, s>>>(dU, grad_weight, row_scale, cout, cin, accumulate);
  DANA_CHECK_LAUNCH("dana_conv3x3_wgrad_winograd4(filter-gradient transform)");
  return DANA_OK;
}

int dana_winograd4_filter_transform(const float* w_packed, float* u, int cout, int cin, dana_stream_t stream) {
  DANA_CHECK_ARG(w_packed && u && cout > 0 && cin > 0, "dana_winograd4_filter_transform: bad args");
  const long total = (long)cout * cin;
  wino4_filter_kernel<<<dana_ceil_div(total, 256), 256, 0, (hipStream_t)stream>>>(w_packed, u, cout, cin);
  DANA_CHECK_LAUNCH("dana_winograd4_filter_transform");
  return DANA_OK;
}

size_t dana_conv3x3_winograd4_workspace_bytes(int batch, int h, int w, int cin, int cout) {
  if (batch <= 0 || h <= 0 || w <= 0 || cin <= 0 || cout <= 0) return 0;
  return wino_plan(batch, h, w, cin, cout, 4).total;
}

static int wino4_impl(const float* input, const float* u, float* output, const float* scale, const float* shift,
                      const float* mask_act, const float* res, long res_pix_stride, int res_group, int batch, int h,
                      int w, int cin, int cout, long in_pix_stride, long out_pix_stride, long mask_pix_stride,
                      int flags, void* workspace, size_t workspace_bytes, dana_stream_t stream, int sub = 1) {
  DANA_CHECK_ARG(batch >= 0 && h > 0 && w > 0 && cin > 0 && cout > 0 && cin % 4 == 0 && cout % 4 == 0,
                 "dana_conv3x3_winograd4_nhwc: bad shape");
  DANA_CHECK_ARG(sub == 1 || (sub == 2 && !mask_act && !res), "dana_conv3x3_winograd4_nhwc: sub is 1 or 2 (2: no mask, no residual)");
  if (batch == 0) return DANA_OK;
  DANA_CHECK_ARG(input && u && output, "dana_conv3x3_winograd4_nhwc: null pointer");
  const long lda = in_pix_stride > 0 ? in_pix_stride : cin;
  const long ldc = out_pix_stride > 0 ? out_pix_stride : cout;
  const long ldm = mask_pix_stride > 0 ? mask_pix_stride : cout;
  const long ldr = res_pix_stride > 0 ? res_pix_stride : cout;
  DANA_CHECK_ARG(!res || (ldr % 4 == 0 && ((uintptr_t)res & 15) == 0 && res_group > 0),
                 "dana_conv3x3_winograd4_nhwc: residual rows must be 16-byte aligned, group > 0");
  DANA_CHECK_ARG(!mask_act || (ldm % 4 == 0 && ((uintptr_t)mask_act & 15) == 0),
                 "dana_conv3x3_winograd4_nhwc: mask rows must be 16-byte aligned");
  DANA_CHECK_ARG(lda % 4 == 0 && ldc % 4 == 0 && ((uintptr_t)input & 15) == 0 && ((uintptr_t)output & 15) == 0,
                 "dana_conv3x3_winograd4_nhwc: strides / pointers must be 16-byte aligned");
  const long in_bytes = (long)batch * h * w * lda * 4;
  DANA_CHECK_ARG(in_bytes < (long)OOB, "dana_conv3x3_winograd4_nhwc: input span >= 2 GiB; split the batch");
  const WinoPlan p = wino_plan(batch, h, w, cin, cout, 4);
  if (!workspace || workspace_bytes < p.total) {
    dana_set_error("dana_conv3x3_winograd4_nhwc: workspace %zu < %zu", workspace_bytes, p.total);
    return DANA_ERR_WORKSPACE;
  }
  hipStream_t s = (hipStream_t)stream;
  float* V = (float*)workspace;
  float* M = (float*)((char*)workspace + p.v_bytes);
  const int C4 = cin / 4, N4 = cout / 4;
  DANA_CHECK_ARG(p.tiles * (long)(C4 > N4 ? C4 : N4) < (1L << 31), "dana_conv3x3_winograd4_nhwc: too many tiles x channels");
  wino4_input_kernel<<<dana_ceil_div(p.tiles * C4, 256), 256, 0, s>>>(input, V, h, w, C4, p.th, p.tw, p.tiles, (int)lda,
                                                                     (unsigned)in_bytes);
  DANA_CHECK_LAUNCH("dana_conv3x3_winograd4_nhwc(input transform)");
  const bool w3 = (flags & DANA_W_SPLIT3) != 0;
  const long kp = (cin + 15) / 16 * 16;
  int rc = dana_gemm_nt(V, u, M, nullptr, nullptr, nullptr, (int)p.tiles, cout, cin, cin, w3 ? kp : cin, cout, 0, 36,
                        p.tiles * cin, w3 ? 3 * cout * kp : (long)cout * cin, p.tiles * cout, 1.f, w3 ? DANA_W_SPLIT3 : 0,
                        stream);
  if (rc) return rc;
  if (sub == 2)
    wino4_output_kernel<2><<<dana_ceil_div(p.tiles * N4, 256), 256, 0, s>>>(M, output, scale, shift, nullptr, ldm, h, w, N4,
                                                                           p.th, p.tw, p.tiles, ldc,
                                                                           (flags & DANA_EPI_RELU) ? 1 : 0);
  else
    wino4_output_kernel<<<dana_ceil_div(p.tiles * N4, 256), 256, 0, s>>>(M, output, scale, shift, mask_act, ldm, h, w, N4,
                                                                        p.th, p.tw, p.tiles, ldc,
                                                                        (flags & DANA_EPI_RELU) ? 1 : 0, 0, 0, res, ldr, res_group);
  DANA_CHECK_LAUNCH("dana_conv3x3_winograd4_nhwc(output transform)");
  return DANA_OK;
}

int dana_conv3x3_winograd4_nhwc_masked(const float* input, const float* u, float* output, const float* scale,
                                       const float* shift, const float* mask_act, int batch, int h, int w, int cin,
                                       int cout, long in_pix_stride, long out_pix_stride, long mask_pix_stride,
                                       int flags, void* workspace, size_t workspace_bytes, dana_stream_t stream) {
  return wino4_impl(input, u, output, scale, shift, mask_act, nullptr, 0, 1, batch, h, w, cin, cout, in_pix_stride,
                    out_pix_stride, mask_pix_stride, flags, workspace, workspace_bytes, stream);
}

int dana_conv3x3_winograd4_nhwc_sub(const float* input, const float* u, float* output, const float* scale,
                                    const float* shift, int batch, int h, int w, int cin, int cout, long in_pix_stride,
                                    long out_pix_stride, int sub, int flags, void* workspace, size_t workspace_bytes,
                                    dana_stream_t stream) {
  return wino4_impl(input, u, output, scale, shift, nullptr, nullptr, 0, 1, batch, h, w, cin, cout, in_pix_stride,
                    out_pix_stride, 0, flags, workspace, workspace_bytes, stream, sub);
}

size_t dana_conv3x3_winograd4_dual_workspace_bytes(int n0, int h0, int w0, int n1, int h1, int w1, int cin, int cout) {
  if (n0 < 0 || n1 < 0 || cin <= 0 || cout <= 0) return 0;
  const long t0 = n0 > 0 ? wino_plan(n0, h0, w0, cin, cout, 4).tiles : 0, t1 = n1 > 0 ? wino_plan(n1, h1, w1, cin, cout, 4).tiles : 0;
  return dana_align_up((size_t)36 * (t0 + t1) * cin * 4, 256) + dana_align_up((size_t)36 * (t0 + t1) * cout * 4, 256);
}

int dana_conv3x3_winograd4_nhwc_dual(const float* input, const float* u, float* out0, float* out1, const float* scale,
                                     const float* shift, int n0, int h0, int w0, int n1, int h1, int w1, int cin,
                                     int cout, long in_pix_stride, long out0_pix_stride, long out1_pix_stride, int flags,
                                     void* workspace, size_t workspace_bytes, dana_stream_t stream) {
  return dana_conv3x3_winograd4_nhwc_dual_masked(input, u, out0, out1, scale, shift, nullptr, nullptr, n0, h0, w0, n1, h1,
                                                 w1, cin, cout, in_pix_stride, out0_pix_stride, out1_pix_stride, 0, 0,
                                                 flags, workspace, workspace_bytes, stream);
}

int dana_conv3x3_winograd4_nhwc_dual_masked(const float* input, const float* u, float* out0, float* out1,
                                            const float* scale, const float* shift, const float* mask0,
                                            const float* mask1, int n0, int h0, int w0, int n1, int h1, int w1, int cin,
                                            int cout, long in_pix_stride, long out0_pix_stride, long out1_pix_stride,
                                            long mask0_pix_stride, long mask1_pix_stride, int flags, void* workspace,
                                            size_t workspace_bytes, dana_stream_t stream) {
  const char* who = "dana_conv3x3_winograd4_nhwc_dual";
  const long ldm0 = mask0_pix_stride > 0 ? mask0_pix_stride : cout, ldm1 = mask1_pix_stride > 0 ? mask1_pix_stride : cout;
  DANA_CHECK_ARG((!mask0 || (ldm0 % 4 == 0 && ((uintptr_t)mask0 & 15) == 0)) && (!mask1 || (ldm1 % 4 == 0 && ((uintptr_t)mask1 & 15) == 0)),
                 "%s: mask rows must be 16-byte aligned", who);
  DANA_CHECK_ARG(n0 > 0 && n1 > 0 && h0 > 0 && w0 > 0 && h1 > 0 && w1 > 0 && cin > 0 && cout > 0 && cin % 4 == 0 && cout % 4 == 0,
                 "%s: bad shape", who);
  DANA_CHECK_ARG(input && u && out0 && out1, "%s: null pointer", who);
  const long lda = in_pix_stride > 0 ? in_pix_stride : cin;
  const long ldc0 = out0_pix_stride > 0 ? out0_pix_stride : cout, ldc1 = out1_pix_stride > 0 ? out1_pix_stride : cout;
  DANA_CHECK_ARG(lda % 4 == 0 && ldc0 % 4 == 0 && ldc1 % 4 == 0 && ((uintptr_t)input & 15) == 0 && ((uintptr_t)out0 & 15) == 0 &&
                     ((uintptr_t)out1 & 15) == 0, "%s: strides / pointers must be 16-byte aligned", who);
  const long in0_bytes = (long)n0 * h0 * w0 * lda * 4, in1_bytes = (long)n1 * h1 * w1 * lda * 4;
  DANA_CHECK_ARG(in0_bytes < (long)OOB && in1_bytes < (long)OOB, "%s: input span >= 2 GiB; split the batch", who);
  const WinoPlan p0 = wino_plan(n0, h0, w0, cin, cout, 4), p1 = wino_plan(n1, h1, w1, cin, cout, 4);
  const long T = p0.tiles + p1.tiles;
  const size_t v_bytes = dana_align_up((size_t)36 * T * cin * 4, 256), need = dana_conv3x3_winograd4_dual_workspace_bytes(n0, h0, w0, n1, h1, w1, cin, cout);
  if (!workspace || workspace_bytes < need) {
    dana_set_error("%s: workspace %zu < %zu", who, workspace_bytes, need);
    return DANA_ERR_WORKSPACE;
  }
  hipStream_t s = (hipStream_t)stream;
  float* V = (float*)workspace;
  float* M = (float*)((char*)workspace + v_bytes);
  const int C4 = cin / 4, N4 = cout / 4;
  DANA_CHECK_ARG(T * (long)(C4 > N4 ? C4 : N4) < (1L << 31), "%s: too many tiles x channels", who);
  const float* in1 = input + (long)n0 * h0 * w0 * lda;
  wino4_input_kernel<<<dana_ceil_div(p0.tiles * C4, 256), 256, 0, s>>>(input, V, h0, w0, C4, p0.th, p0.tw, p0.tiles, (int)lda,
                                                                      (unsigned)in0_bytes, T, 0);
  wino4_input_kernel<<<dana_ceil_div(p1.tiles * C4, 256), 256, 0, s>>>(in1, V, h1, w1, C4, p1.th, p1.tw, p1.tiles, (int)lda,
                                                                      (unsigned)in1_bytes, T, p0.tiles);
  DANA_CHECK_LAUNCH("dana_conv3x3_winograd4_nhwc_dual(input transforms)");
  const bool w3 = (flags & DANA_W_SPLIT3) != 0;
  const long kp = (cin + 15) / 16 * 16;
  int rc = dana_gemm_nt(V, u, M, nullptr, nullptr, nullptr, (int)T, cout, cin, cin, w3 ? kp : cin, cout, 0, 36, T * cin,
                        w3 ? 3 * cout * kp : (long)cout * cin, T * cout, 1.f, w3 ? DANA_W_SPLIT3 : 0, stream);
  if (rc) return rc;
  const int relu = (flags & DANA_EPI_RELU) ? 1 : 0;
  wino4_output_kernel<<<dana_ceil_div(p0.tiles * N4, 256), 256, 0, s>>>(M, out0, scale, shift, mask0, ldm0, h0, w0, N4, p0.th,
                                                                       p0.tw, p0.tiles, ldc0, relu, T, 0);
  wino4_output_kernel<<<dana_ceil_div(p1.tiles * N4, 256), 256, 0, s>>>(M, out1, scale, shift, mask1, ldm1, h1, w1, N4, p1.th,
                                                                       p1.tw, p1.tiles, ldc1, relu, T, p0.tiles);
  DANA_CHECK_LAUNCH("dana_conv3x3_winograd4_nhwc_dual(output transforms)");
  return DANA_OK;
}

int dana_conv3x3_winograd_nhwc_grouped_res(const float* input, const float* u, float* output, const float* scale,
                                           const float* shift, const float* residual, int batch, int h, int w, int cin,
                                           int cout, long in_pix_stride, long out_pix_stride, long res_pix_stride,
                                           int res_group, int tile, int flags, void* workspace, size_t workspace_bytes,
                                           dana_stream_t stream) {
  DANA_CHECK_ARG(residual && res_group > 0 && (tile == 2 || tile == 4),
                 "dana_conv3x3_winograd_nhwc_grouped_res: needs a residual, res_group > 0, tile 2 or 4");
  if (tile == 2)
    return wino2_impl(input, u, output, scale, shift, nullptr, residual, res_pix_stride, res_group, batch, h, w, cin, cout,
                      in_pix_stride, out_pix_stride, 0, flags, workspace, workspace_bytes, stream);
  return wino4_impl(input, u, output, scale, shift, nullptr, residual, res_pix_stride, res_group, batch, h, w, cin, cout,
                    in_pix_stride, out_pix_stride, 0, flags, workspace, workspace_bytes, stream);
}

}
// ... 1 lines not shown
```

dual-awareness-attention-for-few-shot-object-detection_amd/dana.py:

```python
import contextlib
import math
import time
from types import SimpleNamespace

import numpy as np
import torch
import torch.nn as nn
import torch.nn.functional as F

from . import ops
from .config import cfg
from . import targets as T
from .cached_inputs import (BankEpisode, ClassSweep, QueryBank, QueryBatch, SupportBank, SupportCache,
                            check_cached_forward, query_batch_size, query_device, read_inputs, resolve_bank_episode,
                            resolve_query_batch, resolve_shot_views)


class Bottleneck(nn.Module):
    expansion = 4

    def __init__(self, inplanes, planes, stride=1, downsample=None):
        super().__init__()
        self.conv1 = nn.Conv2d(inplanes, planes, kernel_size=1, stride=stride, bias=False)
        self.bn1 = nn.BatchNorm2d(planes)
# ... 25 lines not shown
        self.relu = nn.ReLU(inplace=True)
        self.maxpool = nn.MaxPool2d(kernel_size=3, stride=2, padding=0, ceil_mode=True)
        self.layer1 = _make_layer(64, 64, layers[0], 1)
        self.layer2 = _make_layer(256, 128, layers[1], 2)
        self.layer3 = _make_layer(512, 256, layers[2], 2)
        self.layer4 = _make_layer(1024, 512, layers[3], 2)
        for m in self.modules():
            if isinstance(m, nn.Conv2d):
                n = m.kernel_size[0] * m.kernel_size[1] * m.out_channels
                m.weight.data.normal_(0, math.sqrt(2. / n))
            elif isinstance(m, nn.BatchNorm2d):
                m.weight.data.fill_(1)
                m.bias.data.zero_()


class FFN(nn.Module):

    def __init__(self, in_channel, hidden):
        super().__init__()
        self.linear1 = nn.Linear(in_channel, hidden)
        self.linear2 = nn.Linear(hidden, 2)


class _RPNParams(nn.Module):

    def __init__(self, din):
        super().__init__()
        self.din = din
        self.anchor_scales = cfg.ANCHOR_SCALES
        self.anchor_ratios = cfg.ANCHOR_RATIOS
        self.feat_stride = cfg.FEAT_STRIDE[0]
        self.RPN_Conv = nn.Conv2d(din, 512, 3, 1, 1, bias=True)
        self.nc_score_out = len(self.anchor_scales) * len(self.anchor_ratios) * 2
        self.RPN_cls_score = nn.Conv2d(512, self.nc_score_out, 1, 1, 0)
        self.nc_bbox_out = len(self.anchor_scales) * len(self.anchor_ratios) * 4
        self.RPN_bbox_pred = nn.Conv2d(512, self.nc_bbox_out, 1, 1, 0)


def positional_encoding_table(max_len, d_model=1024):
    pe = torch.zeros(max_len, d_model)
    position = torch.arange(0., max_len).unsqueeze(1)
    div_term = torch.exp(torch.arange(0., d_model, 2) * -(math.log(10000.0) / float(d_model)))
    pe[:, 0::2] = torch.sin(position * div_term)
    pe[:, 1::2] = torch.cos(position * div_term)
    return pe


class _LossBridge(torch.autograd.Function):

    @staticmethod
    def forward(fctx, anchor, model, l1, l2, l3, l4):
        fctx.model = model
        fctx.saved = model._ctx
        return l1.clone(), l2.clone(), l3.clone(), l4.clone()

    @staticmethod
    def backward(fctx, g1, g2, g3, g4):
        from . import backward as BW
        ctx = fctx.saved
        if ctx is None or ctx.get("consumed"):
            raise RuntimeError("the saved activations of this training forward were already consumed by a backward pass "
                               "(each forward can be differentiated once; run the forward again)")
        gs = [torch.zeros((), device=fctx.model._grad_anchor.device) if g is None else g.reshape(()) for g in (g1, g2, g3, g4)]
        fctx.saved = None
        BW.model_backward(fctx.model, torch.stack(gs), ctx=ctx)
        return None, None, None, None, None, None


_HERE = contextlib.nullcontext()

ATTENTION_LEVELS = ("ba", "rpn", "roi")


def _on(stream):
    return _HERE if stream is None else ops.on_stream(stream)


def _rows(t, row):
    return t[row:] if row and t is not None else t


class DAnARCNN(nn.Module):
    trim_strided_seams = True

    def __init__(self, classes, attention_type="concat", rpn_reduce_dim=256, rcnn_reduce_dim=256, gamma=0.1,
                 semantic_enhance=False, num_layers=50, pretrained=False, num_way=2, num_shot=5, pos_encoding=True):
        super().__init__()
        if attention_type not in ("concat", "product"):
            raise ValueError("attention_type must be 'concat' or 'product' (dana.py:70-77)")
        self.model_path = "data/pretrained_model/resnet50_caffe.pth"
        self.dout_base_model = 1024
        self.pretrained = pretrained
        self.classes = classes
        self.n_classes = len(classes)
        self.n_way = num_way
        self.n_shot = num_shot
        self.attention_type = attention_type
        self.channel_gamma = gamma
        self.unary_gamma = 0.1
        self.semantic_enhance = semantic_enhance
        self.rpn_reduce_dim = rpn_reduce_dim
        self.rcnn_reduce_dim = rcnn_reduce_dim
        self.pos_encoding = pos_encoding
        self.pool_feat_dim = 1024
        self.rcnn_dim = 64
        self.use_winograd = True
        self.winograd_tile = 4
        self.winograd_min_cin = 128
        self.presplit_weights = True
        self.merge_trunk = False
        self.merge_from = 0
        self.fold_roi_pe = True
        self.fold_roi_attn = True
        self.prefetch_dgrad = "layer4"
        self.rpn_side_role = "wgrad"
        self.nms_inclusive = False
        dim_in = self.pool_feat_dim

        def lin(i, o):
            m = nn.Linear(i, o)
            nn.init.normal_(m.weight, std=0.01)
            nn.init.constant_(m.bias, 0)
            return m

        self.rpn_unary_layer = lin(dim_in, 1)
        self.rcnn_unary_layer = lin(dim_in, 1)
        self.rpn_adapt_q_layer = lin(dim_in, rpn_reduce_dim)
        self.rpn_adapt_k_layer = lin(dim_in, rpn_reduce_dim)
        self.rcnn_adapt_q_layer = lin(dim_in, rcnn_reduce_dim)
        self.rcnn_adapt_k_layer = lin(dim_in, rcnn_reduce_dim)
        if self.semantic_enhance:
            self.rpn_channel_k_layer = lin(dim_in, 1)
        corr_dim = 2048 if attention_type == "concat" else 1024
        self.RCNN_rpn = _RPNParams(corr_dim)
        self.rcnn_transform_layer = nn.Linear(corr_dim, self.rcnn_dim)
        self.output_score_layer = FFN(64 * 49, dim_in)
        self._plan = None
        self._consts = {}
        self.generalised_support = False
        self.device_rng = False
        self.rng_seed = 1996
        self._rng_calls = 0
        self._conv_cache = {}
        self._epoch = 0
        self._ctx = None
        self._grad_anchor = None

    def create_architecture(self):
        self._init_modules()
        self._init_weights()

    trunk_layers = (3, 4, 6, 3)

    def _init_modules(self):
        resnet = _ResNet50Params(tuple(self.trunk_layers))
        if self.pretrained:
            print("Loading pretrained weights from %s" % (self.model_path))
            state_dict = torch.load(self.model_path)
            resnet.load_state_dict({k: v for k, v in state_dict.items() if k in resnet.state_dict()})
        self.RCNN_base = nn.Sequential(resnet.conv1, resnet.bn1, resnet.relu, resnet.maxpool, resnet.layer1,
                                       resnet.layer2, resnet.layer3)
        self.RCNN_top = nn.Sequential(resnet.layer4)
        self.RCNN_bbox_pred = nn.Linear(2048, 4)
        for p in self.RCNN_base[0].parameters():
            p.requires_grad = False
        for p in self.RCNN_base[1].parameters():
# ... 241 lines not shown
                                     out0=o0, out1=o1, out0_stride=s0, out1_stride=s1, res0_stride=res_stride,
                                     res1_stride=res_stride, stem=stem)
            return o0
        for i, ((n, (h, w), row, st), (o, ld)) in enumerate(zip(segs, dest)):
            with _on(st):
                if wino:
                    ops.conv3x3_winograd(_rows(x, row), n, h, w, cin, b, cout, scale=c["scale"], shift=c["shift"], relu=relu,
                                         in_stride=in_stride, out=o, out_stride=ld,
                                         keep_v=keep[i] if keep is not None else None)
                else:
                    ops.conv2d_nhwc(_rows(x, row), n, h, w, cin, b, cout, k, k, sd, pd, scale=c["scale"], shift=c["shift"],
                                    residual=_rows(res, osegs[i][2]), relu=relu, in_stride=in_stride, out=o, out_stride=ld,
                                    res_stride=res_stride, stem=stem)
        return dest[0][0]

    def _stem(self, segs, ims, c, merged, alloc):
        csegs = self._grid(segs, lambda h, w: ((h - 1) // 2 + 1, (w - 1) // 2 + 1))
        psegs = self._grid(csegs, ops.maxpool_out_size)
        dev = ims[0].device
        x4, xs, xp = (self._dest(g, cols, None, alloc, dev) for g, cols in ((segs, 4), (csegs, 64), (psegs, 64)))
        for g in ([slice(None)] if merged else [slice(i, i + 1) for i in range(len(segs))]):
            for im, (o, _), (_, _, _, st) in zip(ims[g], x4[g], segs[g]):
                with _on(st):
                    ops.nchw_to_nhwc(im, cpad=4, out=o)
            self._conv(segs[g], csegs[g], x4[0][0], c, True, merged, outs=xs[g], stem=True)
            for (n, (h, w), row, st), (o, _) in zip(csegs[g], xp[g]):
                with _on(st):
                    ops.maxpool3x3s2_ceil(_rows(xs[0][0], row), n, h, w, 64, out=o)
        return xp[0][0], psegs

    def _can_trim(self, bp, nbp):
        n1, nds = nbp["c1"], nbp["ds"]
        if nds is None or any((c["k"], c["stride"], c["pad"]) != (1, 2, 0) for c in (n1, nds)):
            return False
        c1, c2, c3 = bp["c1"], bp["c2"], bp["c3"]
        if bp["ds"] is not None or c1["stride"] != 1 or (c2["k"], c2["stride"], c2["pad"]) != (3, 1, 1) or ops.get_mfma_mode() != 1:
            return False
        if c2["cout"] == 64 and c2.get("u") is None and c2["ws"] is not None and c3["ws"] is not None:
            return True
        u = c2.get("u")
        return (u is not None and u.size(0) == 36 and c3["cout"] > 64 and c3["cout"] % 128 == 0
                and ops.get_epilogue_mode() == 0)

    def _block(self, segs, x, bp, merged=False, outs=None, in_stride=0, saves=None, key=None, alloc=None, save_m=None,
               trim=False, pre=False):
        if merged and in_stride:
            raise ValueError("a merged block reads dense rows")
        if saves is not None and saves[0] is None:
            saves = None
        c1, c2, c3, ds = bp["c1"], bp["c2"], bp["c3"], bp["ds"]
        dev, cout, sd = x.device, c3["cout"], 1 if pre else c1["stride"]
        if pre:
            c1, ds = dict(c1, stride=1), dict(ds, stride=1)
        if (trim or pre) and (merged or saves is not None or outs is not None):
            raise ValueError("a trimmed seam: per-segment launches that save nothing and write a fresh buffer")
        osegs = self._grid(segs, lambda h, w: ((h - 1) // sd + 1, (w - 1) // sd + 1))
        calloc = None if merged else alloc
        o1 = self._conv(segs, osegs, x, c1, True, merged, in_stride=in_stride, alloc=calloc)

        def given():
            if outs is None:
                return None
            return [(t if t is not None else alloc(n * h * w, ld) if i and alloc is not None else
                     torch.empty((n * h * w, ld), dtype=torch.float32, device=dev), ld)
                    for i, ((n, (h, w), _, _), (t, ld)) in enumerate(zip(osegs, outs))]

        if (not merged and saves is None and ds is None and c2["cout"] == 64 and c2["k"] == 3 and c2["stride"] == 1
                and c2.get("u") is None and c2["ws"] is not None and c3["ws"] is not None):
            outs = given()
            tsegs = self._grid(osegs, lambda h, w: ((h - 1) // 2 + 1, (w - 1) // 2 + 1)) if trim else osegs
            dest = self._dest(tsegs, cout, outs, calloc, dev)
            for (n, _, row, st), (_, (h1, w1), orow, _), (o, ld) in zip(segs, osegs, dest):
                with _on(st):
                    ops.bottleneck_tail(_rows(o1, orow), n, h1, w1, c2["cin"], c2["ws"], c2["scale"], c2["shift"], c3["ws"],
                                        c3["scale"], c3["shift"], cout, residual=_rows(x, row), res_stride=in_stride, out=o,
                                        out_stride=ld, stride=2 if trim else 1)
            return dest[0][0], tsegs, outs
        if trim:
            tsegs = self._grid(osegs, lambda h, w: ((h - 1) // 2 + 1, (w - 1) // 2 + 1))
            d2, d3 = self._dest(tsegs, c2["cout"], None, calloc, dev), self._dest(tsegs, cout, None, calloc, dev)
            for (n, _, row, st), (_, (h1, w1), orow, _), (_, (h2, w2), _, _), (o2, _), (o, ld) in zip(segs, osegs, tsegs, d2, d3):
                with _on(st):
                    ops.conv3x3_winograd(_rows(o1, orow), n, h1, w1, c2["cin"], c2.get("us") or c2["u"], c2["cout"],
                                         scale=c2["scale"], shift=c2["shift"], relu=True, out=o2, out_stride=c2["cout"], sub=2)
                    ops.conv2d_nhwc(o2, n, h2, w2, c3["cin"], self._b(c3), cout, 1, 1, 1, 0, scale=c3["scale"],
                                    shift=c3["shift"], residual=_rows(x, row), relu=True, out=o, out_stride=ld,
                                    res_stride=in_stride, res_hw=(h1, w1), res_sample=2)
            return d3[0][0], tsegs, None
        keep = [[] for _ in segs] if saves is not None else None
        o2 = self._conv(osegs, osegs, o1, c2, True, merged, keep=keep, alloc=calloc)
        outs = given()
        if bp.get("cat") is not None and ops.get_mfma_mode() != 0:
            cat = bp["cat"]
            dest = self._dest(osegs, cout, outs, calloc, dev)
            if merged:
                (n0, (h0, w0), _, _), (n1, (h1, w1), _, _) = segs
                ops.conv1x1_cat2_dual(o2, c3["cin"], x, ds["cin"], n0, h0, w0, n1, h1, w1, ds["stride"], self._b(cat),
                                      cat["shift"], cout, relu=True, out0=dest[0][0], out1=dest[1][0],
                                      out0_stride=dest[0][1], out1_stride=dest[1][1])
            else:
                for (n, (h, w), row, st), (_, _, orow, _), (o, ld) in zip(segs, osegs, dest):
                    with _on(st):
                        ops.conv1x1_cat2(_rows(o2, orow), c3["cin"], _rows(x, row), ds["cin"], n, h, w, ds["stride"],
                                         self._b(cat), cat["shift"], cout, relu=True, a1_stride=in_stride, out=o, out_stride=ld)
            o3 = dest[0][0]
        else:
            res, rs = x, in_stride
            if ds is not None:
                res, rs = self._conv(segs, osegs, x, ds, False, merged, in_stride=in_stride, alloc=calloc), 0
            o3 = self._conv(osegs, osegs, o2, c3, True, merged, res=res, res_stride=rs, outs=outs, alloc=calloc)
        if saves is not None:
            for i, ((n, (h, w), row, _), (_, (h1, w1), orow, _)) in enumerate(zip(segs, osegs)):
                sx, s1, s2, s3 = x, o1, o2, o3
                if len(segs) > 1:
                    m, mo = n * h * w, n * h1 * w1
                    sx, s1, s2, s3 = x[row:row + m], o1[orow:orow + mo], o2[orow:orow + mo], o3[orow:orow + mo]
                s3, ld = outs[i] if outs is not None else (s3, 0)
                saves[i].append(dict(x=sx, o1=s1, o2=s2, o3=s3, h1=h1, w1=w1, n=n, h=h, w=w, bp=bp, key=key, o3_ld=ld,
                                     v2=keep[i][0] if keep[i] else None))
            if save_m is not None:
                save_m.append(dict(x=x, o1=o1, o2=o2, o3=None if outs is not None else o3, mq_in=segs[1][2],
                                   mq_out=osegs[1][2], m_in=x.size(0), m_out=o1.size(0)))
        return o3, osegs, outs

    def _bottleneck(self, x, n, h, w, bp, out=None, out_stride=0, in_stride=0, save=None, key=None):
        o3, ((_, (h1, w1), _, _),), _ = self._block([(n, (h, w), 0, None)], x, bp, in_stride=in_stride, key=key,
                                                    outs=[(out, out_stride)] if out is not None else None,
                                                    saves=[save])
        return o3, h1, w1

    @staticmethod
    def _drain(gen):
        try:
            while True:
                next(gen)
        except StopIteration as done:
            return done.value

    def _rcnn_base(self, im, plan, out_stride=0, out_buf=None, save=None, save_from=1):
        x, ((_, (h, w), _, _),), _ = self._drain(self._trunk_gen(
            [im], plan, outs=[(out_buf, out_stride)], saves=[save], save_from=save_from))
        return x, h, w

    def _trunk_gen(self, ims, plan, outs=((None, 0),), saves=None, side=None, merge_from=None, save_m=None, save_from=1):
        two, dev = len(ims) > 1, ims[0].device
        alloc = None
        if two:
            main = ops.cur_stream()
            if side == main:
                side = None

            def alloc(rows, cols):
                t = torch.empty((rows, cols), dtype=torch.float32, device=dev)
                if side is not None:
                    t.record_stream(side)
                    ev = torch.cuda.Event()
                    ev.record(main)
                    side.wait_event(ev)
                return t

        def join(segs):
            if side is not None:
                main.wait_event(ops.record_event(side))
            return [(n, hw, row, None) for n, hw, row, _ in segs]

        merged = two and merge_from <= 0
        segs, row = [], 0
# ... 898 lines not shown
```

dual-awareness-attention-for-few-shot-object-detection_amd/ops.py:

```python
import collections
import contextlib
import ctypes
import time as _time

import torch

from ._lib import lib, DanaError

HOST_WAIT = [0.0]

NCHW, NHWC = 0, 1
EPI_RELU, CONV_STEM7, W_SPLIT3, A_SPLIT3 = 1, 2, 256, 512

PROFILE = None
PROF_ROLE = None


def _prof_begin():
    if PROFILE is None:
        return None
    e = torch.cuda.Event(enable_timing=True)
    e.record()
    return e

# ... 655 lines not shown
    return w_cat, shift


def conv1x1_cat2(a0, k0, a1, k1, batch, h1, w1, stride1, w_cat, shift, cout, relu=True, a0_stride=0, a1_stride=0,
                 out=None, out_stride=0):
    _chk(a0, "a0")
    _chk(a1, "a1")
    oh, ow = (h1 - 1) // stride1 + 1, (w1 - 1) // stride1 + 1
    if out is None:
        out = torch.empty((batch * oh * ow, cout), dtype=torch.float32, device=a0.device)
        out_stride = cout
    e0 = _prof_begin()
    wp, wfl = _wf(w_cat)
    lib().call("dana_conv1x1_cat2_nhwc", _p(a0), a0_stride, k0, _p(a1), a1_stride, k1, batch, h1, w1, stride1, wp,
               _p(out), None, _p(shift), None, out_stride, 0, cout, (EPI_RELU if relu else 0) | wfl, _stream())
    m = batch * oh * ow
    _prof_end(e0, ("conv1x1cat M=%d N=%d K=%d s%d", (m, cout, k0 + k1, stride1)), 2.0 * m * cout * (k0 + k1),
              4.0 * (m * (k0 + k1) + cout * (k0 + k1) + m * cout))
    return out, oh, ow


def conv1x1_cat2_dual(a0, k0, a1, k1, n0, h0, w0, n1, h1, w1, stride1, w_cat, shift, cout, relu=True, out0=None,
                      out1=None, out0_stride=0, out1_stride=0):
    _chk(a0, "a0")
    _chk(a1, "a1")
    oh0, ow0 = (h0 - 1) // stride1 + 1, (w0 - 1) // stride1 + 1
    oh1, ow1 = (h1 - 1) // stride1 + 1, (w1 - 1) // stride1 + 1
    m0, m1 = n0 * oh0 * ow0, n1 * oh1 * ow1
    if out0 is None:
        merged = torch.empty((m0 + m1, cout), dtype=torch.float32, device=a0.device)
        out0, out1 = merged, merged[m0:]
        out0_stride = out1_stride = cout
    e0 = _prof_begin()
    wp, wfl = _wf(w_cat)
    lib().call("dana_conv1x1_cat2_nhwc_dual", _p(a0), 0, k0, _p(a1), 0, k1, n0, h0, w0, n1, h1, w1, stride1, wp,
               _p(out0), _p(out1), None, _p(shift), out0_stride, out1_stride, cout, (EPI_RELU if relu else 0) | wfl,
               _stream())
    m = m0 + m1
    _prof_end(e0, ("conv1x1cat M=%d N=%d K=%d s%d", (m, cout, k0 + k1, stride1)), 2.0 * m * cout * (k0 + k1),
              4.0 * (m * (k0 + k1) + cout * (k0 + k1) + m * cout))
    return out0, out1, (oh0, ow0), (oh1, ow1)


def conv3x3_winograd_dual(x, n0, h0, w0, n1, h1, w1, cin, u, cout, scale=None, shift=None, relu=False, mask=None, out=None):
    _chk(x, "x")
    up, wfl = _wf(u)
    if (u.batch if isinstance(u, W3) else u.size(0)) != 36:
        raise ValueError("conv3x3_winograd_dual: F(4x4,3x3) filters only")
    m0, m1 = n0 * h0 * w0, n1 * h1 * w1
    if out is None:
        out = torch.empty((m0 + m1, cout), dtype=torch.float32, device=x.device)
    ws = _ws(lib().query("dana_conv3x3_winograd4_dual_workspace_bytes", n0, h0, w0, n1, h1, w1, cin, cout), x.device)
    e0 = _prof_begin()
    lib().call("dana_conv3x3_winograd4_nhwc_dual_masked", _p(x), up, _p(out), _p(out[m0:]), _p(scale), _p(shift),
               _p(mask), _p(mask[m0:]) if mask is not None else None, n0, h0, w0, n1, h1, w1, cin, cout, 0, 0, 0, 0, 0,
               (EPI_RELU if relu else 0) | wfl, _p(ws), ws.numel(), _stream())
    tiles = n0 * ((h0 + 3) // 4) * ((w0 + 3) // 4) + n1 * ((h1 + 3) // 4) * ((w1 + 3) // 4)
    _prof_end(e0, ("wino3x3 M=%d N=%d K=%d s1", (m0 + m1, cout, 9 * cin)), 2.0 * (m0 + m1) * cout * 9 * cin,
              4.0 * 36 * (tiles * (cin + cout) + cout * cin), executed=2.0 * 36 * tiles * cin * cout)
    return out


def conv3x3_winograd_dual_dgrad(grad_out, n0, h0, w0, n1, h1, w1, cout, ud, cin, mask=None, out=None):
    global PROF_ROLE
    if PROFILE is not None and PROF_ROLE is None:
        PROF_ROLE = "dgrad"
        try:
            return conv3x3_winograd_dual(grad_out, n0, h0, w0, n1, h1, w1, cout, ud, cin, mask=mask, out=out)
        finally:
            PROF_ROLE = None
    return conv3x3_winograd_dual(grad_out, n0, h0, w0, n1, h1, w1, cout, ud, cin, mask=mask, out=out)


def winograd_filter_transform(w_packed, cout, cin, tile=2):
    _chk(w_packed, "w_packed")
    planes = (tile + 2) * (tile + 2)
    u = torch.empty((planes, cout, cin), dtype=torch.float32, device=w_packed.device)
    lib().call("dana_winograd_filter_transform" if tile == 2 else "dana_winograd4_filter_transform", _p(w_packed), _p(u),
               cout, cin, _stream())
    return u


def conv3x3_winograd(x, batch, h, w, cin, u, cout, scale=None, shift=None, relu=False, in_stride=0, out=None,
                     out_stride=0, mask=None, mask_stride=0, keep_v=None, residual=None, res_stride=0, res_group=1, sub=1):
    _chk(x, "x")
    up, wfl = _wf(u)
    m = 2 if (u.batch if isinstance(u, W3) else u.size(0)) == 16 else 4
    if wfl and m != 4:
        raise ValueError("conv3x3_winograd: split filters with F(4x4,3x3) only")
    if sub != 1 and (m != 4 or mask is not None or residual is not None):
        raise ValueError("conv3x3_winograd: sub = 2 needs F(4x4,3x3) filters, no mask, no residual")
    oh, ow = (h - 1) // sub + 1, (w - 1) // sub + 1
    if out is None:
        out = torch.empty((batch * oh * ow, cout), dtype=torch.float32, device=x.device)
        out_stride = cout
    sfx = "" if m == 2 else "4"
    ws = _ws(lib().query("dana_conv3x3_winograd%s_workspace_bytes" % sfx, batch, h, w, cin, cout), x.device)
    e0 = _prof_begin()
    if residual is not None:
        if mask is not None:
            raise ValueError("conv3x3_winograd: a residual and a mask do not combine")
        lib().call("dana_conv3x3_winograd_nhwc_grouped_res", _p(x), up, _p(out), _p(scale), _p(shift),
                   _p(_chk(residual, "residual")), batch, h, w, cin, cout, in_stride, out_stride, res_stride,
                   int(res_group), m, (EPI_RELU if relu else 0) | wfl, _p(ws), ws.numel(), _stream())
    elif sub != 1:
        lib().call("dana_conv3x3_winograd4_nhwc_sub", _p(x), up, _p(out), _p(scale), _p(shift), batch, h, w, cin, cout,
                   in_stride, out_stride, int(sub), (EPI_RELU if relu else 0) | wfl, _p(ws), ws.numel(), _stream())
    else:
        lib().call("dana_conv3x3_winograd%s_nhwc_masked" % sfx, _p(x), up, _p(out), _p(scale), _p(shift), _p(mask), batch,
                   h, w, cin, cout, in_stride, out_stride, mask_stride, (EPI_RELU if relu else 0) | wfl, _p(ws), ws.numel(),
                   _stream())
    if keep_v is not None and m == 4:
        keep_v.append(ws)
    _prof_end(e0, ("wino3x3 M=%d N=%d K=%d s1", (batch * h * w, cout, 9 * cin)), 2.0 * batch * h * w * cout * 9 * cin,
              4.0 * (m + 2) * (m + 2) * (batch * ((h + m - 1) // m) * ((w + m - 1) // m) * (cin + cout) + cout * cin),
              executed=2.0 * (m + 2) * (m + 2) * batch * ((h + m - 1) // m) * ((w + m - 1) // m) * cin * cout)
    return out, oh, ow


def set_mfma_mode(mode):
    prev = lib().query("dana_get_mfma_mode")
    lib().call("dana_set_mfma_mode", int(mode))
    return prev


def get_mfma_mode():
    return lib().query("dana_get_mfma_mode")


def force_tile(tile):
    lib().call("dana_debug_force_tile", int(tile))


def cumask_stream(cus_per_xcd, n_xcd=8, cus_in_xcd=32):
    import ctypes
    words = (n_xcd * cus_in_xcd + 31) // 32
    mask = (ctypes.c_uint * words)()
    for c in cus_per_xcd:
        for x in range(n_xcd):
            i = int(c) * n_xcd + x
            mask[i >> 5] |= 1 << (i & 31)
    out = ctypes.c_void_p()
    lib().call("dana_debug_stream_create_cumask", ctypes.cast(mask, ctypes.c_void_p), words, n_xcd,
               ctypes.cast(ctypes.byref(out), ctypes.c_void_p))
    return torch.cuda.ExternalStream(out.value)


def get_epilogue_mode():
    return lib().query("dana_get_epilogue_mode")


def set_epilogue_mode(mode):
    prev = lib().query("dana_get_epilogue_mode")
    lib().call("dana_set_epilogue_mode", int(mode))
    return prev


def set_dma_kernel(v):
    prev = lib().query("dana_debug_get_dma_kernel")
    lib().call("dana_debug_set_dma_kernel", int(v))
    return prev


def get_dma_kernel():
    return lib().query("dana_debug_get_dma_kernel")


def set_pp_stages(v):
    prev = lib().query("dana_debug_get_pp_stages")
    lib().call("dana_debug_set_pp_stages", int(v))
    return prev


def get_pp_stages():
    return lib().query("dana_debug_get_pp_stages")


IgemmForm = collections.namedtuple("IgemmForm", "family bm bn stem bpre fuse elds nst apre df")
_IGEMM_FAMILIES = {0: None, 1: "f32", 2: "split", 3: "split_128", 4: "dma"}


def decode_igemm_form(code):
    return IgemmForm(_IGEMM_FAMILIES[code & 15], (code >> 4 & 3) * 64, (code >> 6 & 3) * 64, code >> 8 & 1, code >> 9 & 1,
                     code >> 10 & 1, code >> 11 & 1, code >> 12 & 15, code >> 16 & 1, code >> 17 & 1)


def last_igemm_form():
    return decode_igemm_form(lib().query("dana_debug_last_igemm_form"))


@contextlib.contextmanager
def igemm_forms(tile=0, dma=-1, pp=-1, epilogue=0):
    prev_dma, prev_pp, prev_epi = get_dma_kernel(), get_pp_stages(), lib().query("dana_get_epilogue_mode")
    try:
        if tile:
            force_tile(tile)
        set_dma_kernel(dma)
        set_pp_stages(pp)
        set_epilogue_mode(epilogue)
# ... 789 lines not shown
```

include/dana_hip.h:

```cpp
#ifndef DANA_HIP_H
#define DANA_HIP_H
#include <stddef.h>
#include <stdint.h>

#ifdef __cplusplus
extern "C" {
#endif

typedef void* dana_stream_t;

#define DANA_LAYOUT_NCHW 0
#define DANA_LAYOUT_NHWC 1

#define DANA_EPI_RELU 1
#define DANA_CONV_STEM7 2
#define DANA_W_SPLIT3 256
#define DANA_A_SPLIT3 512

const char* dana_last_error(void);
int dana_abi_version(void);

int dana_set_mfma_mode(int mode);
int dana_get_mfma_mode(void);

// ... 68 lines not shown
                          float* gt_boxes, long long* num_boxes, dana_stream_t stream);

int dana_gather_blocks(const void* src_ptrs, const void* dst_ptrs, const long long* block_bytes, int n_tensors,
                       const int* index, int n_sets, int B, dana_stream_t stream);
int dana_gather_shot_blocks(const void* src_ptrs, const void* dst_ptrs, const long long* rows, const long long* block_bytes,
                            int n_tensors, const int* index, const int* view, float* w, int n_sets, int shot, int m, int P,
                            dana_stream_t stream);
int dana_bank_gather_episode(const float* map_pe, const float* pool_pe, const int* index, int n_bank, int B, int way,
                             int shot, int map_rows, int pool_rows, int channels, float* s_pe, float* sp_pe,
                             dana_stream_t stream);
int dana_qbank_gather(const float* maps, const int* index, int n_bank, int B, int rows, int channels, float* out, int ld_out,
                      dana_stream_t stream);

int dana_attn_softmax_unary_sweep(const float* scores, float* out, const float* unary, int B, int C, long hw,
                                  long unary_stride, int nseg, int length, long ld_in, long ld_out, int kpad,
                                  float unary_gamma, float out_scale, dana_stream_t stream);
int dana_attn_softmax_unary_sweep_w(const float* scores, float* out, const float* unary, int B, int C, long hw,
                                    long unary_stride, int nseg, int length, long ld_in, long ld_out, int kpad,
                                    float unary_gamma, const float* seg_scale, long scale_stride, dana_stream_t stream);
int dana_repeat_rows_grouped(const float* src, float* dst, long rows, int cols, long ld_src, long ld_dst, int group,
                             long n_blocks, dana_stream_t stream);
int dana_mul_rows_grouped(float* y, const float* x, long rows, int channels, long ld_y, long ld_x, int group,
                          long n_blocks, dana_stream_t stream);
int dana_meta_class_head(const float* fc7, const float* vec, const float* weight, const float* bias, const float* rois,
                         const float* bbox_pred, float* cls_prob, float* rois_out, float* bbox_out, int B, int C, int R,
                         int K, dana_stream_t stream);
int dana_roi_align_forward_nhwc_grouped(const float* input, const float* rois, float* output, int batch, int channels,
                                        int height, int width, int num_rois, float spatial_scale, int pooled,
                                        int sampling_ratio, long in_pix_stride, long out_pix_stride, float* output2,
                                        const float* add2, long out2_pix_stride, int group, dana_stream_t stream);


int dana_conv2d_nhwc(const float* input, const float* weight, float* output, const float* scale,
                     const float* shift, const float* residual, int batch, int in_h, int in_w, int cin,
                     int cout, int kh, int kw, int stride, int pad, long in_pix_stride, long out_pix_stride,
                     long res_pix_stride, int flags, dana_stream_t stream);

int dana_conv2d_nhwc_masked(const float* input, const float* weight, float* output, const float* scale,
                            const float* shift, const float* residual, const float* mask_act, int batch, int in_h,
                            int in_w, int cin, int cout, int kh, int kw, int stride, int pad, long in_pix_stride,
                            long out_pix_stride, long res_pix_stride, long mask_pix_stride, int flags,
                            dana_stream_t stream);
int dana_bottleneck_tail_nhwc(const float* input, const float* w2_split, const float* scale2, const float* shift2,
                              const float* w3_split, const float* scale3, const float* shift3, const float* residual,
                              float* output, int batch, int h, int w, int cin, int cmid, int cout, long in_pix_stride,
                              long out_pix_stride, long res_pix_stride, int flags, dana_stream_t stream);
int dana_bottleneck_tail_strided_nhwc(const float* input, const float* w2_split, const float* scale2, const float* shift2,
                                      const float* w3_split, const float* scale3, const float* shift3,
                                      const float* residual, float* output, int batch, int h, int w, int cin, int cmid,
                                      int cout, long in_pix_stride, long out_pix_stride, long res_pix_stride, int stride,
                                      int flags, dana_stream_t stream);
int dana_conv2d_nhwc_sampled_res(const float* input, const float* weight, float* output, const float* scale,
                                 const float* shift, const float* residual, int batch, int in_h, int in_w, int cin,
                                 int cout, int kh, int kw, int stride, int pad, long in_pix_stride, long out_pix_stride,
                                 long res_pix_stride, int res_h, int res_w, int res_sample, int flags, dana_stream_t stream);

int dana_conv2d_nhwc_dual(const float* input, const float* weight, float* out0, float* out1, const float* scale,
                          const float* shift, const float* res0, const float* res1, int batch0, int h0, int w0,
                          int batch1, int h1, int w1, int cin, int cout, int kh, int kw, int stride, int pad,
                          long in_pix_stride, long out0_stride, long out1_stride, long res0_stride,
                          long res1_stride, int flags, dana_stream_t stream);

int dana_winograd_filter_transform(const float* w_packed, float* u, int cout, int cin, dana_stream_t stream);
size_t dana_conv3x3_winograd_workspace_bytes(int batch, int h, int w, int cin, int cout);
int dana_conv3x3_winograd_nhwc(const float* input, const float* u, float* output, const float* scale,
                               const float* shift, int batch, int h, int w, int cin, int cout, long in_pix_stride,
                               long out_pix_stride, int flags, void* workspace, size_t workspace_bytes,
                               dana_stream_t stream);
int dana_conv3x3_winograd_nhwc_masked(const float* input, const float* u, float* output, const float* scale,
                                      const float* shift, const float* mask_act, int batch, int h, int w, int cin,
                                      int cout, long in_pix_stride, long out_pix_stride, long mask_pix_stride,
                                      int flags, void* workspace, size_t workspace_bytes, dana_stream_t stream);

int dana_winograd4_filter_transform(const float* w_packed, float* u, int cout, int cin, dana_stream_t stream);
size_t dana_conv3x3_winograd4_workspace_bytes(int batch, int h, int w, int cin, int cout);
int dana_conv3x3_winograd4_nhwc_masked(const float* input, const float* u, float* output, const float* scale,
                                       const float* shift, const float* mask_act, int batch, int h, int w, int cin,
                                       int cout, long in_pix_stride, long out_pix_stride, long mask_pix_stride,
                                       int flags, void* workspace, size_t workspace_bytes, dana_stream_t stream);
int dana_conv3x3_winograd4_nhwc_sub(const float* input, const float* u, float* output, const float* scale,
                                    const float* shift, int batch, int h, int w, int cin, int cout, long in_pix_stride,
                                    long out_pix_stride, int sub, int flags, void* workspace, size_t workspace_bytes,
                                    dana_stream_t stream);
int dana_conv3x3_winograd_nhwc_grouped_res(const float* input, const float* u, float* output, const float* scale,
                                           const float* shift, const float* residual, int batch, int h, int w, int cin,
                                           int cout, long in_pix_stride, long out_pix_stride, long res_pix_stride,
                                           int res_group, int tile, int flags, void* workspace, size_t workspace_bytes,
                                           dana_stream_t stream);
size_t dana_conv3x3_winograd4_dual_workspace_bytes(int n0, int h0, int w0, int n1, int h1, int w1, int cin, int cout);
int dana_conv3x3_winograd4_nhwc_dual(const float* input, const float* u, float* out0, float* out1, const float* scale,
                                     const float* shift, int n0, int h0, int w0, int n1, int h1, int w1, int cin,
                                     int cout, long in_pix_stride, long out0_pix_stride, long out1_pix_stride, int flags,
                                     void* workspace, size_t workspace_bytes, dana_stream_t stream);
int dana_conv3x3_winograd4_nhwc_dual_masked(const float* input, const float* u, float* out0, float* out1,
                                            const float* scale, const float* shift, const float* mask0,
                                            const float* mask1, int n0, int h0, int w0, int n1, int h1, int w1, int cin,
                                            int cout, long in_pix_stride, long out0_pix_stride, long out1_pix_stride,
                                            long mask0_pix_stride, long mask1_pix_stride, int flags, void* workspace,
                                            size_t workspace_bytes, dana_stream_t stream);

size_t dana_conv3x3_wgrad_winograd4_workspace_bytes(int batch, int h, int w, int cin, int cout);
int dana_conv3x3_wgrad_winograd4(const float* grad_out, const float* input, float* grad_weight, int batch, int h, int w,
                                 int cin, int cout, long in_pix_stride, long grad_pix_stride, const float* row_scale,
                                 int accumulate, void* workspace, size_t workspace_bytes, dana_stream_t stream);
int dana_conv3x3_wgrad_winograd4_v(const float* grad_out, const float* v, float* grad_weight, int batch, int h, int w,
                                   int cin, int cout, long grad_pix_stride, const float* row_scale, int accumulate,
                                   void* workspace, size_t workspace_bytes, dana_stream_t stream);

int dana_gemm_nt(const float* a, const float* b, float* c, const float* scale, const float* shift,
                 const float* residual, int m, int n, int k, long lda, long ldb, long ldc, long ldr, int batch,
                 long batch_a, long batch_b, long batch_c, float alpha, int flags, dana_stream_t stream);


int dana_nchw_to_nhwc(const float* in, float* out, int batch, int channels, int height, int width, int cpad,
                      long out_pix_stride, dana_stream_t stream);
int dana_nhwc_to_nchw(const float* in, float* out, int batch, int channels, int height, int width,
                      long in_pix_stride, dana_stream_t stream);
int dana_maxpool3x3s2_ceil_nhwc(const float* in, float* out, int batch, int height, int width, int channels,
                                dana_stream_t stream);
int dana_avgpool_nhwc(const float* in, float* out, int batch, int height, int width, int channels, int k, int stride,
                      dana_stream_t stream);
int dana_spatial_mean_nhwc(const float* in, float* out, int groups, int positions, int channels, long in_pix_stride,
                           dana_stream_t stream);
int dana_batch_stats(const float* x, float* mean, float* var_biased, long rows, int channels, long ld, void* workspace,
                     size_t workspace_bytes, dana_stream_t stream);
int dana_scale_shift_relu(float* x, const float* scale, const float* shift, long rows, int channels, int relu,
                          dana_stream_t stream);
int dana_bn_train_backward(const float* grad_out, const float* x, const float* mean, const float* var_biased,
                           const float* gamma, float eps, long rows, int channels, float* grad_x, float* grad_gamma,
                           float* grad_beta, int accumulate, dana_stream_t stream);
int dana_depthwise_corr_nhwc(const float* feat, const float* kernels, float* out, long n_maps, int height, int width,
                             int channels, int kh, int kw, long maps_per_kernel, long feat_pix_stride,
                             dana_stream_t stream);
int dana_depthwise_corr_nhwc_grouped(const float* feat, const float* kernels, float* out, long n_maps, int height,
                                     int width, int channels, int kh, int kw, int group, long feat_pix_stride,
                                     dana_stream_t stream);
int dana_depthwise_corr_backward_nhwc(const float* grad_out, const float* feat, const float* kernels, float* grad_feat,
                                      float* grad_kernels, long n_maps, int height, int width, int channels, int kh,
                                      int kw, long maps_per_kernel, long feat_pix_stride, int accumulate_kernels,
                                      dana_stream_t stream);
int dana_maxpool2x2s2_nhwc(const float* in, float* out, int batch, int height, int width, int channels,
                           dana_stream_t stream);
int dana_maxpool2x2s2_backward_nhwc(const float* in, const float* grad_out, float* grad_in, int batch, int height,
                                    int width, int channels, dana_stream_t stream);
int dana_sigmoid(float* x, long n, dana_stream_t stream);
int dana_scale_rows_by_group(const float* x, const float* group_vec, float* out, long rows, long rows_per_group,
                             int channels, dana_stream_t stream);
int dana_scale_rows_grouped(const float* x, const float* vec, float* out, long rows, int channels, long ld_x, int group,
                            long n_blocks, dana_stream_t stream);
int dana_add_pe(const float* in, const float* pe, float* out, long rows, int length, int channels,
                long in_stride, long out_stride, dana_stream_t stream);
int dana_add_pe_groups(const float* in, const float* pe, float* out, long groups, long rows_per_group, int length, int channels,
                       long in_group_stride, long out_group_stride, dana_stream_t stream);
size_t dana_colmean_sub_workspace_bytes(int groups, int length, int dim);
int dana_colmean_sub(float* x, int groups, int length, int dim, long ld, void* workspace, size_t workspace_bytes,
                     dana_stream_t stream);
int dana_transpose_batched(const float* in, float* out, int groups, int rows, int cols, long ldi, long ldo,
                           long in_batch, long out_batch, dana_stream_t stream);
int dana_pack_conv_weight(const float* w_oihw, float* out, int cout, int cin, int kh, int kw, int stem7,
                          dana_stream_t stream);
int dana_bn_fold(const float* gamma, const float* beta, const float* mean, const float* var, float eps, float* scale,
                 float* shift, int n, dana_stream_t stream);


int dana_rowdot(const float* x, const float* w, const float* bias, float* out, long rows, int dim, long ld,
                dana_stream_t stream);
int dana_softmax_rows(float* x, long groups, int length, long ld, dana_stream_t stream);
int dana_softmax_rows_to(const float* x, float* out, long groups, int length, long ld_in, long ld_out, dana_stream_t stream);
int dana_labels_posneg_i64(const float* labels, long long* out, long n, dana_stream_t stream);
int dana_ba_apply(float* s, const float* w, int groups, int length, int dim, long ld, float gamma, float slope,
                  dana_stream_t stream);
int dana_attn_softmax_unary(float* scores, const float* unary, long rows, long rows_per_batch, long unary_batch_stride,
                            int nseg, int length, long ld, int kpad, float unary_gamma, float out_scale,
                            dana_stream_t stream);
int dana_attn_softmax_unary_w(float* scores, const float* unary, long rows, long rows_per_batch, long unary_batch_stride,
                              int nseg, int length, long ld, int kpad, float unary_gamma, const float* seg_scale,
                              long scale_batch_stride, dana_stream_t stream);


int dana_proposal_target_prepare(const float* rois, const float* gt_boxes, int B, int n_rois, int n_gt,
                                 float fg_thresh, float bg_thresh_hi, float bg_thresh_lo, float* max_overlaps,
                                 int* gt_assignment, int* fg_list, int* bg_list, int* counts, dana_stream_t stream);
int dana_proposal_target_gather(const float* rois, const float* gt_boxes, int B, int n_rois, int n_gt,
                                const int* gt_assignment, const int* fg_list, const int* bg_list, const int* picks,
                                const int* fg_taken, int rois_per_image, const float* means4, const float* stds4,
                                const float* inside_w4, int normalize, float* rois_out, float* labels_out,
                                float* bbox_targets, float* inside_weights, float* outside_weights,
                                dana_stream_t stream);


int dana_anchor_target_prepare(const float* gt_boxes, const float* im_info, const float* base_anchors, int B,
                               int A, int H, int W, int feat_stride, int n_gt, float negative_overlap,
                               float positive_overlap, float* labels, float* max_overlaps, int* argmax,
                               int* fg_list, int* bg_list, int* counts, dana_stream_t stream);
// ... 200 lines not shown
```

Before: 730.4.

## Skip unused Winograd planes in stride-2 F(4x4,3x3) convolutions via two-level batched GEMM

For stride-2 (sub=2) Winograd F(4x4,3x3) convs, only 25 of the 36 transform planes feed the subsampled outputs. The input transform now writes just those 25 planes, and the per-plane GEMM runs through a new two-level batched launch (batch_inner/batch_skip) that skips the unused plane row and column. This removes roughly 30% of the transform stores and of the batched GEMM work in these convs, at the cost of extra kernel template instantiations. keep_v is rejected when planes are trimmed.

```diff
diff --git a/dual-awareness-attention-for-few-shot-object-detection_amd/csrc/igemm.hip b/dual-awareness-attention-for-few-shot-object-detection_amd/csrc/igemm.hip
--- a/dual-awareness-attention-for-few-shot-object-detection_amd/csrc/igemm.hip
+++ b/dual-awareness-attention-for-few-shot-object-detection_amd/csrc/igemm.hip
@@ -45,6 +45,7 @@
   int res_sample, res_h, res_w, res_oh, res_ow;
   unsigned res_bytes;
   unsigned long long* trace;
+  int batch_inner, batch_skip;
 };
 
 constexpr int BK = 32;
@@ -57,12 +58,18 @@
   return (xcd < r ? xcd * (q + 1) : r * (q + 1) + (xcd - r) * q) + local;
 }
 
+template <int B2>
+__device__ __forceinline__ int batch_slice(const IgemmParams& p, int zb) {
+  if constexpr (B2) return zb + zb / p.batch_inner * p.batch_skip;
+  return zb;
+}
+
 __device__ __forceinline__ float4 ldg_b128(__amdgpu_buffer_rsrc_t r, unsigned off) {
   u32x4 v = __builtin_amdgcn_raw_buffer_load_b128(r, (int)off, 0, 0);
   return *(float4*)&v;
 }
 
-template <int BM, int BN, int STEM>
+template <int BM, int BN, int STEM, int B2 = 0>
 __global__ void __launch_bounds__(256, 2) igemm_f32_kernel(IgemmParams p) {
   constexpr int TM = BM / 64, TN = BN / 64;
   constexpr int RA = BM / 32, RB = BN / 32;
@@ -81,9 +88,10 @@
   const int tile = vid - zb * (int)gridDim.x;
   const int tm_idx = tile / p.tiles_n, tn_idx = tile % p.tiles_n;
   const int m0 = tm_idx * BM, n0 = tn_idx * BN;
-  const float* Ab = p.A + (long)zb * p.batch_a;
-  const float* Bb = p.Bw + (long)zb * p.batch_b;
-  float* Cb = p.C + (long)zb * p.batch_c;
+  const int zs = batch_slice<B2>(p, zb);
+  const float* Ab = p.A + (long)zs * p.batch_a;
+  const float* Bb = p.Bw + (long)zs * p.batch_b;
+  float* Cb = p.C + (long)zs * p.batch_c;
   const __amdgpu_buffer_rsrc_t ra_src = __builtin_amdgcn_make_buffer_rsrc((void*)Ab, 0, (int)p.a_bytes, 0x00020000);
   const __amdgpu_buffer_rsrc_t rb_src = __builtin_amdgcn_make_buffer_rsrc((void*)Bb, 0, (int)p.b_bytes, 0x00020000);
 
@@ -465,7 +473,7 @@
   }
 }
 
-template <int BM, int BN, int STEM, int BPRE = 0, int FUSE = 0, int ELDS = 0, int RSMP = 0>
+template <int BM, int BN, int STEM, int BPRE = 0, int FUSE = 0, int ELDS = 0, int RSMP = 0, int B2 = 0>
 __device__ __forceinline__ void igemm_split_body(const IgemmParams& p) {
   static_assert(!RSMP || (!STEM && !FUSE && !ELDS), "sampled residual: register epilogue of the plain conv / GEMM forms");
   constexpr int TM = BM / 64, TN = BN / 64;
@@ -488,9 +496,10 @@
   const int tile = vid - zb * (int)gridDim.x;
   const int tm_idx = tile / p.tiles_n, tn_idx = tile % p.tiles_n;
   const int m0 = tm_idx * BM, n0 = tn_idx * BN;
-  const float* Ab = p.A + (long)zb * p.batch_a;
-  const float* Bb = p.Bw + (long)zb * p.batch_b;
-  float* Cb = p.C + (long)zb * p.batch_c;
+  const int zs = batch_slice<B2>(p, zb);
+  const float* Ab = p.A + (long)zs * p.batch_a;
+  const float* Bb = p.Bw + (long)zs * p.batch_b;
+  float* Cb = p.C + (long)zs * p.batch_c;
   __amdgpu_buffer_rsrc_t ra_src = __builtin_amdgcn_make_buffer_rsrc((void*)Ab, 0, (int)p.a_bytes, 0x00020000);
   const __amdgpu_buffer_rsrc_t rb_src = __builtin_amdgcn_make_buffer_rsrc((void*)Bb, 0, (int)p.b_bytes, 0x00020000);
 
@@ -1138,16 +1147,16 @@
   }
 }
 
-template <int BM, int BN, int STEM, int BPRE = 0, int FUSE = 0, int ELDS = 0, int RSMP = 0>
+template <int BM, int BN, int STEM, int BPRE = 0, int FUSE = 0, int ELDS = 0, int RSMP = 0, int B2 = 0>
 __global__ void __launch_bounds__(256, 2) igemm_split_kernel(IgemmParams p) {
-  igemm_split_body<BM, BN, STEM, BPRE, FUSE, ELDS, RSMP>(p);
-}
-template <int STEM, int BPRE, int ELDS, int RSMP = 0>
+  igemm_split_body<BM, BN, STEM, BPRE, FUSE, ELDS, RSMP, B2>(p);
+}
+template <int STEM, int BPRE, int ELDS, int RSMP = 0, int B2 = 0>
 __global__ void __launch_bounds__(256, 1) __attribute__((amdgpu_num_vgpr(192))) igemm_split_kernel_128(IgemmParams p) {
-  igemm_split_body<128, 128, STEM, BPRE, 0, ELDS, RSMP>(p);
-}
-
-template <int BN, int NST, int APRE, int DF = 0>
+  igemm_split_body<128, 128, STEM, BPRE, 0, ELDS, RSMP, B2>(p);
+}
+
+template <int BN, int NST, int APRE, int DF = 0, int B2 = 0>
 __global__ void __launch_bounds__(256, NST == 2 ? 3 : (NST == 3 ? 2 : 1)) igemm_dma_kernel(IgemmParams p) {
   static_assert(APRE || NST == 2, "fp32 activation rows: two stages");
   static_assert(!DF || (APRE && NST >= 3), "two fragment sets: planes x planes, three or more stages");
@@ -1169,11 +1178,12 @@
   const int tile = vid - zb * (int)gridDim.x;
   const int tm_idx = tile / p.tiles_n, tn_idx = tile % p.tiles_n;
   const int m0 = tm_idx * BM, n0 = tn_idx * BN;
-  float* Cb = p.C + (long)zb * p.batch_c;
+  const int zs = batch_slice<B2>(p, zb);
+  float* Cb = p.C + (long)zs * p.batch_c;
   __amdgpu_buffer_rsrc_t ra_src =
-      __builtin_amdgcn_make_buffer_rsrc((void*)(p.A + (long)zb * p.batch_a), 0, (int)p.a_bytes, 0x00020000);
+      __builtin_amdgcn_make_buffer_rsrc((void*)(p.A + (long)zs * p.batch_a), 0, (int)p.a_bytes, 0x00020000);
   const __amdgpu_buffer_rsrc_t rb_src =
-      __builtin_amdgcn_make_buffer_rsrc((void*)(p.Bw + (long)zb * p.batch_b), 0, (int)p.b_bytes, 0x00020000);
+      __builtin_amdgcn_make_buffer_rsrc((void*)(p.Bw + (long)zs * p.batch_b), 0, (int)p.b_bytes, 0x00020000);
   const int nk = (p.K + SBK - 1) / SBK;
 
   const int prow = lane >> 1, phalf = (lane & 1) ^ ((lane >> 4) & 1);
@@ -1520,7 +1530,7 @@
   return family | (bm / 64) << 4 | (bn / 64) << 6 | stem << 8 | bpre << 9 | fuse << 10 | elds << 11 | nst << 12 | apre << 16 | df << 17;
 }
 
-template <int BM, int BN, int STEM>
+template <int BM, int BN, int STEM, int B2 = 0>
 int launch(const IgemmParams& p0, int batch, hipStream_t s) {
   g_last_form.store(form_code(DANA_IGEMM_FAMILY_F32, BM, BN, STEM, 0, 0, 0, 0, 0, 0), std::memory_order_relaxed);
   IgemmParams p = p0;
@@ -1530,18 +1540,18 @@
   const size_t lds_c = (size_t)BM * (BN + 4) * sizeof(float);
   if (lds_c > lds) lds = lds_c;
   static DeviceOnce attr;
-  attr.once([&] { return hipFuncSetAttribute((const void*)igemm_f32_kernel<BM, BN, STEM>, hipFuncAttributeMaxDynamicSharedMemorySize, (int)lds); });
+  attr.once([&] { return hipFuncSetAttribute((const void*)igemm_f32_kernel<BM, BN, STEM, B2>, hipFuncAttributeMaxDynamicSharedMemorySize, (int)lds); });
   dim3 grid(p.tiles_m * p.tiles_n, 1, batch);
-  igemm_f32_kernel<BM, BN, STEM><<<grid, 256, lds, s>>>(p);
+  igemm_f32_kernel<BM, BN, STEM, B2><<<grid, 256, lds, s>>>(p);
   return 0;
 }
 
-template <int BM, int BN, int STEM = 0, int BPRE = 0, int FUSE = 0, int ELDS = 0, int RSMP = 0>
+template <int BM, int BN, int STEM = 0, int BPRE = 0, int FUSE = 0, int ELDS = 0, int RSMP = 0, int B2 = 0>
 int launch_split(const IgemmParams& p0, int batch, hipStream_t s) {
   if constexpr (BPRE == 0 && FUSE == 0) {
-    if (p0.bpre) return launch_split<BM, BN, STEM, 1, 0, ELDS, RSMP>(p0, batch, s);
-  }
-  if constexpr (ELDS == 0 && FUSE == 0 && RSMP == 0) {
+    if (p0.bpre) return launch_split<BM, BN, STEM, 1, 0, ELDS, RSMP, B2>(p0, batch, s);
+  }
+  if constexpr (ELDS == 0 && FUSE == 0 && RSMP == 0 && B2 == 0) {
     if (epilogue_mode_cell().load(std::memory_order_relaxed)) return launch_split<BM, BN, STEM, BPRE, 0, 1>(p0, batch, s);
   }
   g_last_form.store(form_code(BM * BN >= 128 * 128 ? DANA_IGEMM_FAMILY_SPLIT_128 : DANA_IGEMM_FAMILY_SPLIT, BM, BN, STEM, BPRE, FUSE ? 1 : 0,
@@ -1557,18 +1567,18 @@
   dim3 grid(p.tiles_m * p.tiles_n, 1, batch);
   static DeviceOnce attr;
   if constexpr (BM * BN >= 128 * 128) {
-    attr.once([&] { return hipFuncSetAttribute((const void*)igemm_split_kernel_128<STEM, BPRE, ELDS, RSMP>, hipFuncAttributeMaxDynamicSharedMemorySize,
+    attr.once([&] { return hipFuncSetAttribute((const void*)igemm_split_kernel_128<STEM, BPRE, ELDS, RSMP, B2>, hipFuncAttributeMaxDynamicSharedMemorySize,
                                 (int)lds); });
-    igemm_split_kernel_128<STEM, BPRE, ELDS, RSMP><<<grid, 256, lds, s>>>(p);
+    igemm_split_kernel_128<STEM, BPRE, ELDS, RSMP, B2><<<grid, 256, lds, s>>>(p);
   } else {
-    attr.once([&] { return hipFuncSetAttribute((const void*)igemm_split_kernel<BM, BN, STEM, BPRE, FUSE, ELDS, RSMP>,
+    attr.once([&] { return hipFuncSetAttribute((const void*)igemm_split_kernel<BM, BN, STEM, BPRE, FUSE, ELDS, RSMP, B2>,
                                 hipFuncAttributeMaxDynamicSharedMemorySize, (int)lds); });
-    igemm_split_kernel<BM, BN, STEM, BPRE, FUSE, ELDS, RSMP><<<grid, 256, lds, s>>>(p);
+    igemm_split_kernel<BM, BN, STEM, BPRE, FUSE, ELDS, RSMP, B2><<<grid, 256, lds, s>>>(p);
   }
   return 0;
 }
 
-template <int BN, int NST, int APRE, int DF = 0>
+template <int BN, int NST, int APRE, int DF = 0, int B2 = 0>
 int launch_dma(const IgemmParams& p0, int batch, hipStream_t s) {
   g_last_form.store(form_code(DANA_IGEMM_FAMILY_DMA, 128, BN, 0, 1, 0, 0, NST, APRE, DF), std::memory_order_relaxed);
   IgemmParams p = p0;
@@ -1576,9 +1586,9 @@
   p.tiles_n = (p.N + BN - 1) / BN;
   const size_t lds = (size_t)NST * 3 * (128 + BN) * 32;
   static DeviceOnce attr;
-  attr.once([&] { return hipFuncSetAttribute((const void*)igemm_dma_kernel<BN, NST, APRE, DF>, hipFuncAttributeMaxDynamicSharedMemorySize, (int)lds); });
+  attr.once([&] { return hipFuncSetAttribute((const void*)igemm_dma_kernel<BN, NST, APRE, DF, B2>, hipFuncAttributeMaxDynamicSharedMemorySize, (int)lds); });
   dim3 grid(p.tiles_m * p.tiles_n, 1, batch);
-  igemm_dma_kernel<BN, NST, APRE, DF><<<grid, 256, lds, s>>>(p);
+  igemm_dma_kernel<BN, NST, APRE, DF, B2><<<grid, 256, lds, s>>>(p);
   return 0;
 }
 
@@ -1625,7 +1635,19 @@
   return launch_split<128, 128, 0, 0, 0, 0, 1>(p, batch, s);
 }
 
+int dispatch_batch2(const IgemmParams& p, int batch, hipStream_t s) {
+  const int mode = mfma_mode_cell().load(std::memory_order_relaxed);
+  if (p.apre || p.mask || p.residual || p.res_sample) return -1;
+  if (!mode) return launch<64, 64, 0, 1>(p, batch, s);
+  const long t128 = (long)((p.M + 127) / 128) * ((p.N + 127) / 128) * batch;
+  if (p.bpre && p.N > 64 && t128 >= 600 && p.K <= 192) return launch_dma<128, 2, 0, 0, 1>(p, batch, s);
+  if (p.N <= 64) return launch_split<128, 64, 0, 0, 0, 0, 0, 1>(p, batch, s);
+  if (t128 < 100) return launch_split<64, 64, 0, 0, 0, 0, 0, 1>(p, batch, s);
+  return launch_split<128, 128, 0, 0, 0, 0, 0, 1>(p, batch, s);
+}
+
 int dispatch(const IgemmParams& p, int batch, int stem, hipStream_t s) {
+  if (p.batch_inner) return stem ? -1 : dispatch_batch2(p, batch, s);
   if (p.res_sample) return stem ? -1 : dispatch_sampled(p, batch, s);
   if (stem) {
     const int smode = mfma_mode_cell().load(std::memory_order_relaxed);
@@ -2069,9 +2091,10 @@
   return DANA_OK;
 }
 
-int dana_gemm_nt(const float* a, const float* b, float* c, const float* scale, const float* shift,
-                 const float* residual, int m, int n, int k, long lda, long ldb, long ldc, long ldr, int batch,
-                 long batch_a, long batch_b, long batch_c, float alpha, int flags, dana_stream_t stream) {
+static int gemm_nt_impl(const float* a, const float* b, float* c, const float* scale, const float* shift,
+                        const float* residual, int m, int n, int k, long lda, long ldb, long ldc, long ldr, int batch,
+                        long batch_a, long batch_b, long batch_c, float alpha, int flags, dana_stream_t stream,
+                        int batch_inner, int batch_outer_step) {
   DANA_CHECK_ARG(m >= 0 && n >= 0 && k > 0 && batch >= 0, "dana_gemm_nt: bad shape m=%d n=%d k=%d", m, n, k);
   if (m == 0 || n == 0 || batch == 0) return DANA_OK;
   DANA_CHECK_ARG(a && b && c, "dana_gemm_nt: null pointer");
@@ -2126,12 +2149,32 @@
   p.apre = apre;
   p.a_rows = m;
   p.batch_c = batch_c;
+  p.batch_inner = batch_inner;
+  p.batch_skip = batch_inner ? batch_outer_step - batch_inner : 0;
   p.bpre = bpre;
   p.alpha = alpha;
   p.relu = (flags & DANA_EPI_RELU) ? 1 : 0;
-  run(p, batch, 0, s);
+  const int rc = run(p, batch, 0, s);
+  DANA_CHECK_ARG(!batch_inner || rc == 0, "dana_gemm_nt_batch2: no kernel form takes this launch (planes x planes operands)");
   DANA_CHECK_LAUNCH("dana_gemm_nt");
   return DANA_OK;
 }
 
-}
+int dana_gemm_nt(const float* a, const float* b, float* c, const float* scale, const float* shift,
+                 const float* residual, int m, int n, int k, long lda, long ldb, long ldc, long ldr, int batch,
+                 long batch_a, long batch_b, long batch_c, float alpha, int flags, dana_stream_t stream) {
+  return gemm_nt_impl(a, b, c, scale, shift, residual, m, n, k, lda, ldb, ldc, ldr, batch, batch_a, batch_b, batch_c, alpha,
+                      flags, stream, 0, 0);
+}
+
+int dana_gemm_nt_batch2(const float* a, const float* b, float* c, const float* scale, const float* shift, int m, int n,
+                        int k, long lda, long ldb, long ldc, int batch_inner, int batch_outer, int batch_outer_step,
+                        long batch_a, long batch_b, long batch_c, float alpha, int flags, dana_stream_t stream) {
+  DANA_CHECK_ARG(batch_inner > 0 && batch_outer >= 0 && batch_outer_step >= batch_inner &&
+                     (long)batch_inner * batch_outer < (1L << 16),
+                 "dana_gemm_nt_batch2: needs batch_inner > 0, batch_outer >= 0, batch_outer_step >= batch_inner");
+  return gemm_nt_impl(a, b, c, scale, shift, nullptr, m, n, k, lda, ldb, ldc, 0, batch_inner * batch_outer, batch_a, batch_b,
+                      batch_c, alpha, flags, stream, batch_inner, batch_outer_step);
+}
+
+}
diff --git a/dual-awareness-attention-for-few-shot-object-detection_amd/csrc/winograd.hip b/dual-awareness-attention-for-few-shot-object-detection_amd/csrc/winograd.hip
--- a/dual-awareness-attention-for-few-shot-object-detection_amd/csrc/winograd.hip
+++ b/dual-awareness-attention-for-few-shot-object-detection_amd/csrc/winograd.hip
@@ -4,6 +4,7 @@
 namespace {
 
 typedef unsigned int u32x4 __attribute__((ext_vector_type(4)));
+typedef float f32x4 __attribute__((ext_vector_type(4)));
 constexpr unsigned OOB = 0x80000000u;
 
 __device__ __forceinline__ float4 f4add(float4 a, float4 b) { return make_float4(a.x + b.x, a.y + b.y, a.z + b.z, a.w + b.w); }
@@ -185,6 +186,7 @@
   }
 }
 
+template <bool LIVE25 = false>
 __global__ void __launch_bounds__(256)
 wino4_input_kernel(const float* __restrict__ in, float* __restrict__ V, int H, int W, int C4, int th, int tw,
                    long tiles, int lda, unsigned in_bytes, long plane_tiles = 0, long tile_off = 0) {
@@ -217,12 +219,21 @@
   }
   const long plane = plane_tiles * (long)C4;
   float4* out = (float4*)V + (tile_off + t) * C4 + c4;
-#pragma unroll
-  for (int r = 0; r < 6; ++r) {
+  constexpr int LIVE = LIVE25 ? 5 : 6;
+#pragma unroll
+  for (int r = 0; r < LIVE; ++r) {
     float4 o[6];
     bt6(tm[r], o);
 #pragma unroll
-    for (int c = 0; c < 6; ++c) out[(r * 6 + c) * plane] = o[c];
+    for (int c = 0; c < LIVE; ++c) {
+      if constexpr (LIVE25) {
+        f32x4 q = {o[c].x, o[c].y, o[c].z, o[c].w};
+        asm volatile("" : "+v"(q));
+        *(f32x4*)&out[(r * 6 + c) * plane] = q;
+      } else {
+        out[(r * 6 + c) * plane] = o[c];
+      }
+    }
   }
 }
 
@@ -553,10 +564,12 @@
 static int wino4_impl(const float* input, const float* u, float* output, const float* scale, const float* shift,
                       const float* mask_act, const float* res, long res_pix_stride, int res_group, int batch, int h,
                       int w, int cin, int cout, long in_pix_stride, long out_pix_stride, long mask_pix_stride,
-                      int flags, void* workspace, size_t workspace_bytes, dana_stream_t stream, int sub = 1) {
+                      int flags, void* workspace, size_t workspace_bytes, dana_stream_t stream, int sub = 1,
+                      bool all_planes = true) {
   DANA_CHECK_ARG(batch >= 0 && h > 0 && w > 0 && cin > 0 && cout > 0 && cin % 4 == 0 && cout % 4 == 0,
                  "dana_conv3x3_winograd4_nhwc: bad shape");
   DANA_CHECK_ARG(sub == 1 || (sub == 2 && !mask_act && !res), "dana_conv3x3_winograd4_nhwc: sub is 1 or 2 (2: no mask, no residual)");
+  const bool live25 = sub == 2 && !all_planes;
   if (batch == 0) return DANA_OK;
   DANA_CHECK_ARG(input && u && output, "dana_conv3x3_winograd4_nhwc: null pointer");
   const long lda = in_pix_stride > 0 ? in_pix_stride : cin;
@@ -581,14 +594,21 @@
   float* M = (float*)((char*)workspace + p.v_bytes);
   const int C4 = cin / 4, N4 = cout / 4;
   DANA_CHECK_ARG(p.tiles * (long)(C4 > N4 ? C4 : N4) < (1L << 31), "dana_conv3x3_winograd4_nhwc: too many tiles x channels");
-  wino4_input_kernel<<<dana_ceil_div(p.tiles * C4, 256), 256, 0, s>>>(input, V, h, w, C4, p.th, p.tw, p.tiles, (int)lda,
-                                                                     (unsigned)in_bytes);
+  if (live25)
+    wino4_input_kernel<true><<<dana_ceil_div(p.tiles * C4, 256), 256, 0, s>>>(input, V, h, w, C4, p.th, p.tw, p.tiles,
+                                                                             (int)lda, (unsigned)in_bytes);
+  else
+    wino4_input_kernel<<<dana_ceil_div(p.tiles * C4, 256), 256, 0, s>>>(input, V, h, w, C4, p.th, p.tw, p.tiles, (int)lda,
+                                                                       (unsigned)in_bytes);
   DANA_CHECK_LAUNCH("dana_conv3x3_winograd4_nhwc(input transform)");
   const bool w3 = (flags & DANA_W_SPLIT3) != 0;
   const long kp = (cin + 15) / 16 * 16;
-  int rc = dana_gemm_nt(V, u, M, nullptr, nullptr, nullptr, (int)p.tiles, cout, cin, cin, w3 ? kp : cin, cout, 0, 36,
-                        p.tiles * cin, w3 ? 3 * cout * kp : (long)cout * cin, p.tiles * cout, 1.f, w3 ? DANA_W_SPLIT3 : 0,
-                        stream);
+  int rc = live25 ? dana_gemm_nt_batch2(V, u, M, nullptr, nullptr, (int)p.tiles, cout, cin, cin, w3 ? kp : cin, cout, 5, 5, 6,
+                                        p.tiles * cin, w3 ? 3 * cout * kp : (long)cout * cin, p.tiles * cout, 1.f,
+                                        w3 ? DANA_W_SPLIT3 : 0, stream)
+                  : dana_gemm_nt(V, u, M, nullptr, nullptr, nullptr, (int)p.tiles, cout, cin, cin, w3 ? kp : cin, cout, 0,
+                                 36, p.tiles * cin, w3 ? 3 * cout * kp : (long)cout * cin, p.tiles * cout, 1.f,
+                                 w3 ? DANA_W_SPLIT3 : 0, stream);
   if (rc) return rc;
   if (sub == 2)
     wino4_output_kernel<2><<<dana_ceil_div(p.tiles * N4, 256), 256, 0, s>>>(M, output, scale, shift, nullptr, ldm, h, w, N4,
@@ -615,7 +635,15 @@
                                     long out_pix_stride, int sub, int flags, void* workspace, size_t workspace_bytes,
                                     dana_stream_t stream) {
   return wino4_impl(input, u, output, scale, shift, nullptr, nullptr, 0, 1, batch, h, w, cin, cout, in_pix_stride,
-                    out_pix_stride, 0, flags, workspace, workspace_bytes, stream, sub);
+                    out_pix_stride, 0, flags, workspace, workspace_bytes, stream, sub, false);
+}
+
+int dana_conv3x3_winograd4_nhwc_sub_planes(const float* input, const float* u, float* output, const float* scale,
+                                           const float* shift, int batch, int h, int w, int cin, int cout,
+                                           long in_pix_stride, long out_pix_stride, int sub, int all_planes, int flags,
+                                           void* workspace, size_t workspace_bytes, dana_stream_t stream) {
+  return wino4_impl(input, u, output, scale, shift, nullptr, nullptr, 0, 1, batch, h, w, cin, cout, in_pix_stride,
+                    out_pix_stride, 0, flags, workspace, workspace_bytes, stream, sub, all_planes != 0);
 }
 
 size_t dana_conv3x3_winograd4_dual_workspace_bytes(int n0, int h0, int w0, int n1, int h1, int w1, int cin, int cout) {
diff --git a/dual-awareness-attention-for-few-shot-object-detection_amd/dana.py b/dual-awareness-attention-for-few-shot-object-detection_amd/dana.py
--- a/dual-awareness-attention-for-few-shot-object-detection_amd/dana.py
+++ b/dual-awareness-attention-for-few-shot-object-detection_amd/dana.py
@@ -131,6 +131,7 @@
 
 class DAnARCNN(nn.Module):
     trim_strided_seams = True
+    trim_winograd_planes = True
 
     def __init__(self, classes, attention_type="concat", rpn_reduce_dim=256, rcnn_reduce_dim=256, gamma=0.1,
                  semantic_enhance=False, num_layers=50, pretrained=False, num_way=2, num_shot=5, pos_encoding=True):
@@ -538,7 +539,8 @@
             for (n, _, row, st), (_, (h1, w1), orow, _), (_, (h2, w2), _, _), (o2, _), (o, ld) in zip(segs, osegs, tsegs, d2, d3):
                 with _on(st):
                     ops.conv3x3_winograd(_rows(o1, orow), n, h1, w1, c2["cin"], c2.get("us") or c2["u"], c2["cout"],
-                                         scale=c2["scale"], shift=c2["shift"], relu=True, out=o2, out_stride=c2["cout"], sub=2)
+                                         scale=c2["scale"], shift=c2["shift"], relu=True, out=o2, out_stride=c2["cout"], sub=2,
+                                         all_planes=not self.trim_winograd_planes)
                     ops.conv2d_nhwc(o2, n, h2, w2, c3["cin"], self._b(c3), cout, 1, 1, 1, 0, scale=c3["scale"],
                                     shift=c3["shift"], residual=_rows(x, row), relu=True, out=o, out_stride=ld,
                                     res_stride=in_stride, res_hw=(h1, w1), res_sample=2)
diff --git a/dual-awareness-attention-for-few-shot-object-detection_amd/ops.py b/dual-awareness-attention-for-few-shot-object-detection_amd/ops.py
--- a/dual-awareness-attention-for-few-shot-object-detection_amd/ops.py
+++ b/dual-awareness-attention-for-few-shot-object-detection_amd/ops.py
@@ -761,7 +761,8 @@
 
 
 def conv3x3_winograd(x, batch, h, w, cin, u, cout, scale=None, shift=None, relu=False, in_stride=0, out=None,
-                     out_stride=0, mask=None, mask_stride=0, keep_v=None, residual=None, res_stride=0, res_group=1, sub=1):
+                     out_stride=0, mask=None, mask_stride=0, keep_v=None, residual=None, res_stride=0, res_group=1, sub=1,
+                     all_planes=False):
     _chk(x, "x")
     up, wfl = _wf(u)
     m = 2 if (u.batch if isinstance(u, W3) else u.size(0)) == 16 else 4
@@ -769,6 +770,8 @@
         raise ValueError("conv3x3_winograd: split filters with F(4x4,3x3) only")
     if sub != 1 and (m != 4 or mask is not None or residual is not None):
         raise ValueError("conv3x3_winograd: sub = 2 needs F(4x4,3x3) filters, no mask, no residual")
+    if sub != 1 and not all_planes and keep_v is not None:
+        raise ValueError("conv3x3_winograd: sub = 2 writes 25 of V's 36 planes; keep_v needs all_planes=True")
     oh, ow = (h - 1) // sub + 1, (w - 1) // sub + 1
     if out is None:
         out = torch.empty((batch * oh * ow, cout), dtype=torch.float32, device=x.device)
@@ -783,17 +786,19 @@
                    _p(_chk(residual, "residual")), batch, h, w, cin, cout, in_stride, out_stride, res_stride,
                    int(res_group), m, (EPI_RELU if relu else 0) | wfl, _p(ws), ws.numel(), _stream())
     elif sub != 1:
-        lib().call("dana_conv3x3_winograd4_nhwc_sub", _p(x), up, _p(out), _p(scale), _p(shift), batch, h, w, cin, cout,
-                   in_stride, out_stride, int(sub), (EPI_RELU if relu else 0) | wfl, _p(ws), ws.numel(), _stream())
+        lib().call("dana_conv3x3_winograd4_nhwc_sub_planes", _p(x), up, _p(out), _p(scale), _p(shift), batch, h, w, cin,
+                   cout, in_stride, out_stride, int(sub), int(bool(all_planes)), (EPI_RELU if relu else 0) | wfl, _p(ws),
+                   ws.numel(), _stream())
     else:
         lib().call("dana_conv3x3_winograd%s_nhwc_masked" % sfx, _p(x), up, _p(out), _p(scale), _p(shift), _p(mask), batch,
                    h, w, cin, cout, in_stride, out_stride, mask_stride, (EPI_RELU if relu else 0) | wfl, _p(ws), ws.numel(),
                    _stream())
     if keep_v is not None and m == 4:
         keep_v.append(ws)
+    planes = 25 if sub == 2 and not all_planes else (m + 2) * (m + 2)
     _prof_end(e0, ("wino3x3 M=%d N=%d K=%d s1", (batch * h * w, cout, 9 * cin)), 2.0 * batch * h * w * cout * 9 * cin,
-              4.0 * (m + 2) * (m + 2) * (batch * ((h + m - 1) // m) * ((w + m - 1) // m) * (cin + cout) + cout * cin),
-              executed=2.0 * (m + 2) * (m + 2) * batch * ((h + m - 1) // m) * ((w + m - 1) // m) * cin * cout)
+              4.0 * planes * (batch * ((h + m - 1) // m) * ((w + m - 1) // m) * (cin + cout) + cout * cin),
+              executed=2.0 * planes * batch * ((h + m - 1) // m) * ((w + m - 1) // m) * cin * cout)
     return out, oh, ow
 
 
diff --git a/include/dana_hip.h b/include/dana_hip.h
--- a/include/dana_hip.h
+++ b/include/dana_hip.h
@@ -174,6 +174,10 @@
                                     const float* shift, int batch, int h, int w, int cin, int cout, long in_pix_stride,
                                     long out_pix_stride, int sub, int flags, void* workspace, size_t workspace_bytes,
                                     dana_stream_t stream);
+int dana_conv3x3_winograd4_nhwc_sub_planes(const float* input, const float* u, float* output, const float* scale,
+                                           const float* shift, int batch, int h, int w, int cin, int cout,
+                                           long in_pix_stride, long out_pix_stride, int sub, int all_planes, int flags,
+                                           void* workspace, size_t workspace_bytes, dana_stream_t stream);
 int dana_conv3x3_winograd_nhwc_grouped_res(const float* input, const float* u, float* output, const float* scale,
                                            const float* shift, const float* residual, int batch, int h, int w, int cin,
                                            int cout, long in_pix_stride, long out_pix_stride, long res_pix_stride,
@@ -202,6 +206,9 @@
 int dana_gemm_nt(const float* a, const float* b, float* c, const float* scale, const float* shift,
                  const float* residual, int m, int n, int k, long lda, long ldb, long ldc, long ldr, int batch,
                  long batch_a, long batch_b, long batch_c, float alpha, int flags, dana_stream_t stream);
+int dana_gemm_nt_batch2(const float* a, const float* b, float* c, const float* scale, const float* shift, int m, int n,
+                        int k, long lda, long ldb, long ldc, int batch_inner, int batch_outer, int batch_outer_step,
+                        long batch_a, long batch_b, long batch_c, float alpha, int flags, dana_stream_t stream);
 
 
 int dana_nchw_to_nhwc(const float* in, float* out, int batch, int channels, int height, int width, int cpad,
```

After: 733.9 (median of 6 runs). No clear change (+0.5%).
